# neggles/neurosis

Measured on AMD Instinct MI355X. Metric: train images/sec (node) SDXL 1024^2, higher is better.
Workload: dtype bf16

## Files before the change

include/neurosis_hip.h:

```cpp
#ifndef NEUROSIS_HIP_H
#define NEUROSIS_HIP_H

#ifdef __cplusplus
extern "C" {
#endif

const char* nk_last_error(void);
int nk_abi_version(void);

int nk_linear_fwd(const void* x, const void* w, const float* bias, const void* residual, void* y,
                  int M, int N, int K, long ldx, long ldw, long ldr, long ldy, float alpha, void* stream);
int nk_linear_dgrad(const void* dy, const void* w, const void* dx_add, void* dx, int M, int N, int K,
                    long lddy, long ldw, long ldadd, long lddx, void* stream);
long nk_linear_fwd_geglu_ok(int M, int I, int K);
int nk_linear_fwd_geglu(const void* x, const void* w, const float* bias, void* u, void* h, int M, int I, int K, long ldx, long ldw, long ldu,
                        long ldh, void* stream);
int nk_linear_dgrad_geglu(const void* dy, const void* w, const void* u, void* du, int M, int N, int I, long lddy, long ldw, long ldu,
                          long lddu, void* stream);
int nk_linear_fwd_geglu_s(const void* x, const void* w, const float* bias, void* s, void* h, int M, int I, int K, long ldx, long ldw, long lds,
                          long ldh, void* stream);
int nk_linear_dgrad_geglu_s(const void* dy, const void* w, const void* s, void* du, int M, int N, int I, long lddy, long ldw, long lds,
                            long lddu, void* stream);
int nk_linear_wgrad(const void* dy, const void* x, float* dw, int M, int N, int K, long lddy, long ldx,
                    long lddw, int accumulate, void* stream);
int nk_linear_wgrad_bias(const void* dy, const void* x, float* dw, float* dbias, int M, int N, int K, long lddy, long ldx, long lddw,
                         int accumulate, void* stream);

int nk_gemm_sk_status(void);

int nk_health_status(void);
int nk_health_clear(void);
int nk_health_export(int* dst, void* stream);
int nk_health_import(const int* src, void* stream);
int nk_debug_raise_health(void* stream);
int nk_debug_stamp(unsigned long long* dst, void* stream);
int nk_debug_launch_log(int mode);
long nk_debug_launch_names(char* buf, long cap);

int nk_colsum_batched(const void* dy, float* out, float* ws, long M, int N, long ld, int nbatch, int accumulate, void* stream);

int nk_linear_fwd_batched(const void* const* x, const void* const* w, void* const* y, int count, int M, int N, int K,
                          long ldx, long ldw, long ldy, void* stream);

int nk_linear_wgrad_batched(const void* const* dy, const void* const* x, float* const* dw, float* const* dbias, int count, int M, int N,
                            int K, long lddy, long ldx, long lddw, int accumulate, void* stream);

typedef struct NkConvDesc {
  int N, H, W, Cin;
  int Cout, KH, KW;
  int stride;
  int pad_t, pad_l;
  int Ho, Wo;
  int upsample;
} NkConvDesc;
int nk_conv2d_fwd(const NkConvDesc* d, const void* x, const void* w, const float* bias, const void* rowvec,
                  const void* residual, void* y, void* stream);
long nk_conv2d_stats_tiles(const NkConvDesc* d, int stats_groups);
int nk_conv2d_fwd_stats(const NkConvDesc* d, const void* x, const void* w, const float* bias, const void* rowvec, const void* residual,
                        void* y, float* stats_part, int stats_groups, void* stream);
int nk_conv3x3_few_channels_fwd(const void* x, const void* w, const float* bias, void* y, int N, int H, int W, int Cout, int cin_real,
                                void* stream);
int nk_conv_weight_flip(const void* w, void* wt, int Cout, int Cin, int taps, void* stream);
long nk_conv2d_dgrad_flipped_ok(const NkConvDesc* d);
int nk_conv2d_dgrad_flipped(const NkConvDesc* d, const void* dy, const void* wt, void* dx, void* stream);
int nk_conv2d_dgrad(const NkConvDesc* d, const void* dy, const void* w, void* dx, void* stream);
int nk_conv2d_wgrad(const NkConvDesc* d, const void* dy, const void* x, float* dw, int accumulate, void* stream);
int nk_conv2d_wgrad_bias(const NkConvDesc* d, const void* dy, const void* x, float* dw, float* dbias, int accumulate, void* stream);

int nk_up2_phase_weights(const void* w, void* wp, void* wd, int Cout, int Cin, void* stream);
long nk_conv2d_up2_ws_bytes(const NkConvDesc* d, int direction);
int nk_conv2d_up2_fwd(const NkConvDesc* d, const void* x, const void* wp, const float* bias, void* y, void* ws, void* stream);
int nk_conv2d_up2_dgrad(const NkConvDesc* d, const void* dy, const void* wd, void* dx, void* stream);
int nk_conv2d_up2_wgrad(const NkConvDesc* d, const void* dy, const void* x, float* dw, int accumulate, void* ws, void* stream);
int nk_conv2d_up2_wgrad_bias(const NkConvDesc* d, const void* dy, const void* x, float* dw, float* dbias, int accumulate, void* ws, void* stream);
int nk_pixel_shuffle2x(const void* phases, void* y, int N, int H, int W, int C, void* stream);
int nk_pixel_unshuffle2x(const void* y, void* phases, int N, int H, int W, int C, void* stream);
int nk_up2_fold_wgrad(const float* dwp, const float* dbias_p, float* dw, float* dbias, int Cout, int Cin, int accumulate, void* stream);

typedef struct NkAttnDesc {
  int B, H, Lq, Lk, D;
  long sq, sk, sv, so;
  long bq, bk, bv, bo;
  long sdq, sdk, sdv, sdo;
  long bdq, bdk, bdv, bdo;
  float scale;
  int causal;
} NkAttnDesc;
int nk_attention_fwd(const NkAttnDesc* d, const void* q, const void* k, const void* v, void* o, float* lse,
                     void* stream);
long nk_attention_bwd_ws_floats(const NkAttnDesc* d);
int nk_attention_bwd(const NkAttnDesc* d, const void* q, const void* k, const void* v, const void* o,
                     const float* lse, const void* d_o, void* dq, void* dk, void* dv, float* delta_ws, void* stream);
int nk_attention_bwd_causal(const NkAttnDesc* d, const void* q, const void* k, const void* v, const void* o,
                            const float* lse, const void* d_o, void* dq, void* dk, void* dv, void* stream);
int nk_attention_relbias_fwd(const NkAttnDesc* d, const void* q, const void* k, const void* v, void* o, const float* rel, void* stream);
int nk_attention_relbias_fwd_lse(const NkAttnDesc* d, const void* q, const void* k, const void* v, void* o, float* lse, const float* rel, void* stream);
long nk_attention_relbias_bwd_ws_floats(const NkAttnDesc* d);
int nk_attention_relbias_bwd(const NkAttnDesc* d, const void* q, const void* k, const void* v, const void* o, const float* lse, const void* d_o, void* dq,
                             void* dk, void* dv, const float* rel, float* d_rel, float* ws, int accumulate, void* stream);
int nk_relbias_bucket_sum(const float* d_rel, const int* buckets, float* d_weight, int H, int L, int num_buckets, int accumulate, void* stream);
int nk_softmax_rows(void* s, long M, int L, void* stream);

long nk_groupnorm_ws_floats(int N, int HW, int C, int G);
int nk_groupnorm_fwd(const void* x, const float* gamma, const float* beta, void* y, float* mean, float* rstd,
                     float* ws, int N, int HW, int C, int G, float eps, int silu, void* stream);
int nk_groupnorm_sums(const void* x, float* sums, float* ws, int N, int HW, int C, int G, void* stream);
long nk_groupnorm_sums_ws_floats(int N, int nparts, int G);
int nk_groupnorm_sums_from_parts(const float* part, float* sums, float* ws, int N, int nparts, int G, void* stream);
int nk_groupnorm_apply(const void* x, const float* sums, const float* gamma, const float* beta, void* y, float* mean, float* rstd,
                       int N, int HW, int C, int G, float eps, int silu, void* stream);
int nk_groupnorm_bwd(const void* dy, const void* x, const float* gamma, const float* beta, const float* mean,
                     const float* rstd, const void* dx_add, void* dx, float* dgamma, float* dbeta, float* ws,
                     int N, int HW, int C, int G, int silu, int accumulate, void* stream);
int nk_groupnorm_mod_fwd(const void* x, const float* gamma, const float* beta, const void* mod, void* y, float* mean, float* rstd,
                         float* ws, int N, int HW, int C, int G, float eps, int silu, void* stream);
int nk_groupnorm_mod_apply(const void* x, const float* sums, const float* gamma, const float* beta, const void* mod, void* y, float* mean,
                           float* rstd, int N, int HW, int C, int G, float eps, int silu, void* stream);
int nk_groupnorm_mod_bwd(const void* dy, const void* x, const float* gamma, const float* beta, const void* mod, const float* mean,
                         const float* rstd, const void* dx_add, void* dx, float* dgamma, float* dbeta, void* dmod, float* ws,
                         int N, int HW, int C, int G, int silu, int accumulate, void* stream);

int nk_layernorm_fwd(const void* x, const float* gamma, const float* beta, void* y, float* mean, float* rstd,
                     int M, int C, float eps, void* stream);
long nk_layernorm_ws_floats(int M, int C);
int nk_rmsnorm_fwd(const void* x, const float* gamma, void* y, int M, int C, float eps, void* stream);
int nk_rmsnorm_fwd_rstd(const void* x, const float* gamma, void* y, float* rstd, int M, int C, float eps, void* stream);
long nk_rmsnorm_bwd_ws_floats(int M, int C);
int nk_rmsnorm_bwd(const void* dy, const void* x, const float* gamma, const float* rstd, const void* dx_add, void* dx, float* dgamma, float* ws, int M, int C,
                   int accumulate, void* stream);
int nk_layernorm_bwd(const void* dy, const void* x, const float* gamma, const float* mean, const float* rstd,
                     const void* dx_add, void* dx, float* dgamma, float* dbeta, float* ws, int M, int C, int accumulate, void* stream);
#define NK_COLPART_MAX 32
typedef struct NkColpartBatch {
  const float* part[NK_COLPART_MAX];
  float* dgamma[NK_COLPART_MAX];
  float* dbeta[NK_COLPART_MAX];
  int nrows[NK_COLPART_MAX];
  int C[NK_COLPART_MAX];
  int accumulate[NK_COLPART_MAX];
  int n;
} NkColpartBatch;
long nk_layernorm_part_rows(int M);
int nk_layernorm_bwd_rows(const void* dy, const void* x, const float* gamma, const float* mean, const float* rstd,
                          const void* dx_add, void* dx, float* part, int M, int C, void* stream);
int nk_colpart_reduce_batch(const NkColpartBatch* b, void* stream);
int nk_layernorm_bwd_dx(const void* dy, const void* x, const float* gamma, const float* mean, const float* rstd,
                        const void* dx_add, void* dx, int M, int C, void* stream);
int nk_layernorm_bwd_params(const void* dy, const void* x, const float* mean, const float* rstd, float* dgamma,
                            float* dbeta, float* ws, int M, int C, int accumulate, void* stream);

int nk_geglu_fwd(const void* u, void* y, long M, int I, void* stream);
int nk_geglu_bwd(const void* dy, const void* u, void* du, long M, int I, void* stream);
int nk_geglu_fwd_s(const void* u, void* y, void* s, long M, int I, void* stream);
int nk_geglu_bwd_s(const void* dy, const void* s, void* du, long M, int I, void* stream);

int nk_silu_fwd(const void* x, void* y, long n, void* stream);
int nk_silu_bwd(const void* dy, const void* x, void* dx, long n, void* stream);

int nk_dropout(const void* x, const void* residual, void* y, long rows, int cols, long ld_x, long ld_res, long ld_y, const void* token,
               int site, int thr, float scale, void* stream);
int nk_dropout_draw(void* state, void* token, void* stream);

int nk_add(const void* a, const void* b, void* out, long n, void* stream);

int nk_cat_channels(const void* a, const void* b, void* out, long rows, int Ca, int Cb, void* stream);
int nk_split_channels(const void* src, void* a, void* b, long rows, int Ca, int Cb, void* stream);

int nk_upsample2x_bwd(const void* dup, void* dx, int N, int H, int W, int C, void* stream);
int nk_upsample2x_fwd(const void* x, void* up, int N, int H, int W, int C, void* stream);
int nk_avgpool2x_fwd(const void* x, void* y, int N, int H, int W, int C, void* stream);
int nk_avgpool2x_bwd(const void* dy, void* dx, int N, int H, int W, int C, void* stream);

int nk_nchw_to_nhwc(const void* src, int src_is_f32, void* dst, int N, int C, int HW, int Cpad, float scale,
                    void* stream);
int nk_nhwc_to_nchw(const void* src, void* dst, int dst_is_f32, int N, int C, int HW, int Cpad, void* stream);
int nk_cast_f32_to_bf16(const float* src, void* dst, long n, void* stream);
int nk_cast_bf16_to_f32(const void* src, float* dst, long n, void* stream);

long nk_colsum_ws_floats(long M, int N);
int nk_colsum(const void* dy, float* out, float* ws, long M, int N, long ld, int accumulate, void* stream);

int nk_softmax_rows_bwd(const void* p, void* dp, long M, int L, float scale, void* stream);

int nk_leaky_relu_fwd(const void* x, void* y, long n, float slope, void* stream);
int nk_leaky_relu_bwd(const void* dy, const void* y, void* dx, long n, float slope, void* stream);
long nk_batchnorm_ws_floats(long M, int C);
int nk_batchnorm_fwd(const void* x, const float* gamma, const float* beta, void* y, float* mean, float* rstd, float* running_mean,
                     float* running_var, float* ws, long M, int C, float eps, float momentum, float slope, void* stream);
int nk_batchnorm_bwd(const void* dy, const void* x, const void* y, const float* gamma, const float* mean, const float* rstd, void* dx,
                     float* dgamma, float* dbeta, float* ws, long M, int C, float slope, int accumulate, void* stream);
int nk_batchnorm_eval(const void* x, const float* gamma, const float* beta, const float* running_mean, const float* running_var, void* y,
                      float* ws, long M, int C, float eps, float slope, void* stream);

int nk_maxpool2x2_fwd(const void* x, void* y, int N, int H, int W, int C, void* stream);
int nk_maxpool2x2_bwd(const void* dy, const void* x, void* dx, int N, int H, int W, int C, void* stream);
int nk_maxpool_fwd(const void* x, void* y, int N, int H, int W, int C, int k, int s, void* stream);
// ... 124 lines not shown
```

neurosis_amd/csrc/conv_halo.h:

```cpp
#pragma once
#include <type_traits>

#ifdef NK_HALO_STAMPS
__device__ unsigned long long nk_halo_stamp_buf[8 * 8192];
__device__ unsigned long long nk_halo_kstep_buf[3 * 16 * 20 * 5];
#define CH_KSTAMP(t, ph) do { const int w_ = tid >> 6; if ((tid & 63) == 0 && (w_ == 0 || w_ == 4 || w_ == 6) && blockIdx.x >= 2048 && blockIdx.x < 2048 + 16 && (t) < 20) \
    nk_halo_kstep_buf[((((w_ == 0 ? 0 : (w_ == 4 ? 1 : 2)) * 16 + (blockIdx.x - 2048)) * 20 + (t)) * 5) + (ph)] = __builtin_amdgcn_s_memtime(); } while (0)
extern "C" int nk_debug_halo_ksteps(unsigned long long* host_out) {
  return hipMemcpyFromSymbol(host_out, HIP_SYMBOL(nk_halo_kstep_buf), sizeof(nk_halo_kstep_buf)) == hipSuccess ? 0 : 1;
}
#define CH_STAMP(slot) do { if (tid == 0 && blockIdx.x < 8192) nk_halo_stamp_buf[blockIdx.x * 8 + (slot)] = __builtin_amdgcn_s_memtime(); } while (0)
#define CH_STAMP_RT(slot) do { if (tid == 0 && blockIdx.x < 8192) nk_halo_stamp_buf[blockIdx.x * 8 + (slot)] = __builtin_amdgcn_s_memrealtime(); } while (0)
extern "C" int nk_debug_halo_stamps(unsigned long long* host_out, int nwg) {
  return hipMemcpyFromSymbol(host_out, HIP_SYMBOL(nk_halo_stamp_buf), (size_t)nwg * 8 * sizeof(unsigned long long)) == hipSuccess ? 0 : 1;
}
#else
#define CH_STAMP(slot)
#define CH_STAMP_RT(slot)
#define CH_KSTAMP(t, ph)
#endif
template <int BN_> struct HaloRing {
  static constexpr bool DEEP = BN_ == 128;
  static constexpr int BST = DEEP ? CH_BSTAGE_DEEP : CH_BSTAGE;
  static constexpr int NS = DEEP ? CH_NS_DEEP : CH_NS;
// ... 209 lines not shown
  unsigned so = 0, sn = R::AHEAD * R::BST;
  int t = 0;
  int sl = s0;
  for (int s = 0; s < nslab; ++s) {
    const unsigned hcur = lds0 + (unsigned)(s & 1) * HBUF;
    char* const hnext = smem + ((s + 1) & 1) * HBUF;
    const bool more = s + 1 < nslab;
    const int sln = sl + 1 == nslab ? 0 : sl + 1;
    const long adv_end = sl + 1 == nslab ? adv_wrap : adv_slab;
    auto step = [&](auto tapc) {
      constexpr int tap = decltype(tapc)::value;
      constexpr int dy = tap / 3, dx = tap % 3;
      __builtin_amdgcn_sched_barrier(0);
      int hpv = hpl;
      asm volatile("" : "+v"(hpv));
      g2_read<OP_KC, BN_, NJ>(bfr, fb, so);
#pragma unroll
      for (int r = 0; r < RPW; ++r) {
        const int hp = hpv + (r + dy) * CH_HW + dx;
        const unsigned ar = (unsigned)(hp * 128 + ((cl4 ^ (hp & 7)) << 4));
        const unsigned a0 = hcur + ar, a1 = hcur + (ar ^ 64u);
        G2_RD128(af[2 * r], a0, 0);
        G2_RD128(af[2 * r + 1], a0, 2048);
        G2_RD128(af[MI + 2 * r], a1, 0);
        G2_RD128(af[MI + 2 * r + 1], a1, 2048);
      }
      if constexpr (PROD) {
      } else if (hwave) {
        if (more) {
          constexpr int cnt = ch_count(HPW, HLAST, tap), st = ch_start(HPW, HLAST, tap);
#pragma unroll
          for (int i = 0; i < cnt; ++i) fire_halo(st + i, sln, hnext);
        }
        if (tap == 8) asm volatile("s_waitcnt vmcnt(0)" ::: "memory");
      } else {
        asm volatile("s_waitcnt vmcnt(0)" ::: "memory");
      }
      CH_KSTAMP(t, 4);
      CH_BAR();
      CH_KSTAMP(t, 0);
      asm volatile("s_waitcnt lgkmcnt(0)" ::: "memory");
      __builtin_amdgcn_sched_barrier(0);
      __builtin_amdgcn_s_setprio(1);
      if constexpr (!PROD) {
        if (!hwave) {
          constexpr int tap2 = (tap + 2) % 9;
          wb.fire_next(t + 2 < nk, tap2 == 8 ? adv_end : adv_tap, ring + sn, wave);
        }
      }
      CH_KSTAMP(t, 1);
#pragma unroll
      for (int ks = 0; ks < 2; ++ks)
#pragma unroll
        for (int i = 0; i < MI; ++i)
#pragma unroll
          for (int j = 0; j < NJ; ++j)
            acc[i][j] = __builtin_amdgcn_mfma_f32_16x16x32_bf16(bfr[ks * NJ + j], af[ks * MI + i], acc[i][j], 0, 0, 0);
      __builtin_amdgcn_s_setprio(0);
      CH_KSTAMP(t, 2);
      CH_BAR();
      CH_KSTAMP(t, 3);
      so += R::BST; if (so == R::NS * R::BST) so = 0;
      sn += R::BST; if (sn == R::NS * R::BST) sn = 0;
      ++t;
    };
    step(std::integral_constant<int, 0>{}); step(std::integral_constant<int, 1>{}); step(std::integral_constant<int, 2>{});
    step(std::integral_constant<int, 3>{}); step(std::integral_constant<int, 4>{}); step(std::integral_constant<int, 5>{});
    step(std::integral_constant<int, 6>{}); step(std::integral_constant<int, 7>{}); step(std::integral_constant<int, 8>{});
    sl = sln;
  }
  if (grp == 0) { CH_BAR(); }
  asm volatile("s_waitcnt vmcnt(0)" ::: "memory");
  CH_STAMP(2); CH_STAMP_RT(5);

  int mrow[MI];
  bool mok[MI];
#pragma unroll
  for (int i = 0; i < MI; ++i) {
    const int y = y0 + wq * RPW + (i >> 1), x = x0 + (i & 1) * 16 + (lane & 15);
    mok[i] = y < H && x < W;
    mrow[i] = (img * H + y) * W + x;
  }
  bf16_t* const C = (bf16_t*)p.C;
  uint4_t res8[MI][NJ / 2 ? NJ / 2 : 1];
  uint2_t res4[MI];
  if (p.residual) {
#pragma unroll
    for (int i = 0; i < MI; ++i) {
#pragma unroll
      for (int h = 0; h < NJ / 2; ++h) {
        const int n = nb + h * 32 + (g4 & 1) * 16 + (g4 >> 1) * 8;
        res8[i][h] = (mok[i] && n < Cout) ? *(const uint4_t*)(p.residual + (long)mrow[i] * p.ldr + n) : (uint4_t){0u, 0u, 0u, 0u};
      }
      if constexpr (NJ & 1) {
        const int n = nb + (NJ - 1) * 16 + g4 * 4;
        res4[i] = (mok[i] && n < Cout) ? *(const uint2_t*)(p.residual + (long)mrow[i] * p.ldr + n) : (uint2_t){0u, 0u};
      }
    }
  }
  float cadd[NJ / 2][8], cadd4[4];
#pragma unroll
  for (int h = 0; h < NJ / 2; ++h) {
    const int n = nb + h * 32 + (g4 & 1) * 16 + (g4 >> 1) * 8;
#pragma unroll
    for (int e = 0; e < 8; ++e) cadd[h][e] = 0.f;
    if (n < Cout) {
      if (p.bias) {
        const float4_t b0 = *(const float4_t*)(p.bias + n), b1 = *(const float4_t*)(p.bias + n + 4);
        cadd[h][0] = b0[0]; cadd[h][1] = b0[1]; cadd[h][2] = b0[2]; cadd[h][3] = b0[3];
        cadd[h][4] = b1[0]; cadd[h][5] = b1[1]; cadd[h][6] = b1[2]; cadd[h][7] = b1[3];
      }
      if (p.rowvec) {
        float t[8];
        unpack8(*(const uint4_t*)(p.rowvec + (long)img * p.ld_rowvec + n), t);
#pragma unroll
        for (int e = 0; e < 8; ++e) cadd[h][e] += t[e];
      }
    }
  }
#pragma unroll
  for (int e = 0; e < 4; ++e) cadd4[e] = 0.f;
  if constexpr (NJ & 1) {
    const int n = nb + (NJ - 1) * 16 + g4 * 4;
    if (n < Cout) {
      if (p.bias) { const float4_t b = *(const float4_t*)(p.bias + n); cadd4[0] = b[0]; cadd4[1] = b[1]; cadd4[2] = b[2]; cadd4[3] = b[3]; }
      if (p.rowvec) {
        float t[4];
        unpack4(*(const uint2_t*)(p.rowvec + (long)img * p.ld_rowvec + n), t);
        cadd4[0] += t[0]; cadd4[1] += t[1]; cadd4[2] += t[2]; cadd4[3] += t[3];
      }
    }
  }

  float st8[NJ / 2 ? NJ / 2 : 1][8][2], st4[4][2];
  if constexpr (STATS) {
#pragma unroll
    for (int h = 0; h < NJ / 2; ++h)
#pragma unroll
      for (int e = 0; e < 8; ++e) { st8[h][e][0] = 0.f; st8[h][e][1] = 0.f; }
#pragma unroll
    for (int e = 0; e < 4; ++e) { st4[e][0] = 0.f; st4[e][1] = 0.f; }
  }
#pragma unroll
  for (int i = 0; i < MI; ++i) {
#pragma unroll
    for (int h = 0; h < NJ / 2; ++h) {
      float v[8];
#pragma unroll
      for (int r = 0; r < 4; ++r) {
        const float a_own = acc[i][2 * h][r], b_own = acc[i][2 * h + 1][r];
        auto sw = __builtin_amdgcn_permlane16_swap(__float_as_uint(a_own), __float_as_uint(b_own), false, false);
        v[r] = __uint_as_float(sw[0]);
        v[4 + r] = __uint_as_float(sw[1]);
      }
      const int n = nb + h * 32 + (g4 & 1) * 16 + (g4 >> 1) * 8;
#pragma unroll
      for (int e = 0; e < 8; ++e) v[e] += cadd[h][e];
      if (p.residual) {
        float tr[8];
        unpack8(res8[i][h], tr);
#pragma unroll
        for (int e = 0; e < 8; ++e) v[e] += tr[e];
      }
      const uint4_t packed = pack8(v);
      const bool ok = mok[i] && n < Cout;
      if (ok) *(uint4_t*)(C + (long)mrow[i] * p.ldc + n) = packed;
      if constexpr (STATS) {
        float q[8];
        unpack8(packed, q);
#pragma unroll
        for (int e = 0; e < 8; ++e) { const float x = ok ? q[e] : 0.f; st8[h][e][0] += x; st8[h][e][1] += x * x; }
      }
    }
    if constexpr (NJ & 1) {
      const int n = nb + (NJ - 1) * 16 + g4 * 4;
      float v[4] = {acc[i][NJ - 1][0] + cadd4[0], acc[i][NJ - 1][1] + cadd4[1], acc[i][NJ - 1][2] + cadd4[2], acc[i][NJ - 1][3] + cadd4[3]};
      if (p.residual) {
        float tr[4];
        unpack4(res4[i], tr);
        v[0] += tr[0]; v[1] += tr[1]; v[2] += tr[2]; v[3] += tr[3];
      }
      uint2_t o;
      o.x = pack2bf(v[0], v[1]);
      o.y = pack2bf(v[2], v[3]);
      const bool ok = mok[i] && n < Cout;
      if (ok) *(uint2_t*)(C + (long)mrow[i] * p.ldc + n) = o;
      if constexpr (STATS) {
        float q[4];
        unpack4(o, q);
#pragma unroll
        for (int e = 0; e < 4; ++e) { const float x = ok ? q[e] : 0.f; st4[e][0] += x; st4[e][1] += x * x; }
      }
    }
  }
  if constexpr (STATS) {
    __syncthreads();
    float* const cs = (float*)ring;
    auto lane16_sum = [](float x) {
      x += __builtin_bit_cast(float, __builtin_amdgcn_update_dpp(0, __builtin_bit_cast(int, x), 0xB1, 0xF, 0xF, true));
      x += __builtin_bit_cast(float, __builtin_amdgcn_update_dpp(0, __builtin_bit_cast(int, x), 0x4E, 0xF, 0xF, true));
      x += __builtin_bit_cast(float, __builtin_amdgcn_update_dpp(0, __builtin_bit_cast(int, x), 0x141, 0xF, 0xF, true));
      x += __builtin_bit_cast(float, __builtin_amdgcn_update_dpp(0, __builtin_bit_cast(int, x), 0x140, 0xF, 0xF, true));
      return x;
    };
#pragma unroll
    for (int h = 0; h < NJ / 2; ++h)
#pragma unroll
      for (int e = 0; e < 8; ++e)
#pragma unroll
        for (int k = 0; k < 2; ++k) {
          const float tot = lane16_sum(st8[h][e][k]);
          const int col = h * 32 + (g4 & 1) * 16 + (g4 >> 1) * 8 + e;
          if ((lane & 15) == 0) cs[(wave * HN + col) * 2 + k] = tot;
        }
    if constexpr (NJ & 1) {
#pragma unroll
      for (int e = 0; e < 4; ++e)
#pragma unroll
        for (int k = 0; k < 2; ++k) {
          const float tot = lane16_sum(st4[e][k]);
          const int col = (NJ - 1) * 16 + g4 * 4 + e;
          if ((lane & 15) == 0) cs[(wave * HN + col) * 2 + k] = tot;
        }
    }
    __syncthreads();
    const int cpg = Cout / p.stats_groups;
    const int ngt = BN_ / cpg;
    if (tid < 2 * ngt) {
      const int gi = tid >> 1, k = tid & 1;
      float a = 0.f;
      for (int cc = 0; cc < cpg; ++cc) {
        const int col = gi * cpg + cc;
        const int gh = col / HN, cl = col - gh * HN;
#pragma unroll
        for (int w4 = 0; w4 < 4; ++w4) a += cs[((gh * 4 + w4) * HN + cl) * 2 + k];
      }
      p.stats_part[((long)img * per_img + trem) * 2 * p.stats_groups + 2 * (n0 / cpg + gi) + k] = a;
    }
  }
#ifdef NK_HALO_STAMPS
  asm volatile("s_waitcnt vmcnt(0)" ::: "memory");
  CH_STAMP(3);
#endif
#undef CH_BAR
}
```

neurosis_amd/csrc/gemm.hip:

```cpp
#include "nk_common.h"
#include "nk_gemm.h"
#include "gemm_plan.h"

#define NTHREADS 256
#define KC_IMAGE_BYTES (128 * 128)
#define MC_ROW_BYTES (128 * 2 + 16)
#define MC_IMAGE_BYTES (BK * MC_ROW_BYTES)
#define OPND_BYTES MC_IMAGE_BYTES
#define STAGE_BYTES (2 * OPND_BYTES)
#define SMEM_BYTES (2 * STAGE_BYTES)

static_assert(SMEM_BYTES >= BM * CS_LD * 4, "epilogue staging must fit");

__device__ __forceinline__ bool is_kc(int mode) { return mode == OP_KC || mode == OP_KCG; }

__device__ __forceinline__ long gather_offset(const NkGather& g, int n, int bh, int bw, int kh, int kw,
                                              int c, bool& valid) {
  int hn = bh + kh * g.ks;
  int wn = bw + kw * g.ks;
  bool ok = (hn >= 0) & (wn >= 0);
  ok &= (((hn | wn) & g.need_even) == 0);
  const int sh = g.div >> 1;
  int h = hn >> sh, w = wn >> sh;
  ok &= (h < g.H) & (w < g.W);
// ... 1306 lines not shown
    for (int q = 0; q < 2; ++q) {
      ba[q] = p.bias ? *(const float4_t*)(p.bias + abase + q * 16 + cl) : (float4_t){0.f, 0.f, 0.f, 0.f};
      bg[q] = p.bias ? *(const float4_t*)(p.bias + I + abase + q * 16 + cl) : (float4_t){0.f, 0.f, 0.f, 0.f};
    }
    NkGemmParams ph = p;
    ph.N = I; ph.ldc = p.ld_h; ph.bias = nullptr;
    NkGemmParams ps = p;
    ps.bias = nullptr;
#pragma unroll
    for (int ib = 0; ib < 2; ++ib) {
      float4_t pa[4][2], pg[4][2], phh[4][2];
#pragma unroll
      for (int i = 0; i < 4; ++i)
#pragma unroll
        for (int q = 0; q < 2; ++q) {
          pa[i][q] = acc[ib * 4 + i][2 * q];
          pg[i][q] = acc[ib * 4 + i][2 * q + 1];
#pragma unroll
          for (int r = 0; r < 4; ++r) {
            const float av = bf2f(f2bf(pa[i][q][r] + ba[q][r])), gv = bf2f(f2bf(pg[i][q][r] + bg[q][r]));
            float cdf, pdf;
            normal_cdf_pdf(gv, cdf, pdf);
            const float ge = gv * cdf;
            phh[i][q][r] = av * ge;
            if (p.geglu_save) {
              pa[i][q][r] = ge;
              pg[i][q][r] = av * (cdf + gv * pdf);
            }
          }
        }
      const int mb = m0 + wm * 128 + ib * 64;
      if (p.geglu_save) {
        reg_epilogue_64x32<0>(ps, p.C, pa, mb, abase, lane);
        reg_epilogue_64x32<0>(ps, p.C, pg, mb, I + abase, lane);
      } else {
        reg_epilogue_64x32<0>(p, p.C, pa, mb, abase, lane);
        reg_epilogue_64x32<0>(p, p.C, pg, mb, I + abase, lane);
      }
      reg_epilogue_64x32<0>(ph, p.geglu_h, phh, mb, abase, lane);
    }
    return;
  }
#pragma unroll
  for (int ib = 0; ib < 2; ++ib)
#pragma unroll
    for (int half = 0; half < 2; ++half) {
      float4_t pair[4][2];
#pragma unroll
      for (int i = 0; i < 4; ++i) { pair[i][0] = acc[ib * 4 + i][2 * half]; pair[i][1] = acc[ib * 4 + i][2 * half + 1]; }
      reg_epilogue_64x32<0>(p, p.C, pair, m0 + wm * 128 + ib * 64, n0 + wn * 64 + half * 32, lane);
    }
}

__global__ void nk_zero_f32_kernel(float* __restrict__ dst, size_t n);
#include "gemm_g2.h"
#include "gemm_w160.h"
#include "conv_halo.h"
#include "conv_wgrad_halo.h"

typedef void (*NkGemmKernel)(const NkGemmParams);
static int launch_plan(NkGemmKernel kern, const NkGemmPlan& pl, const NkGemmParams& p, hipStream_t stream) {
  nk_optin_lds((const void*)kern, pl.smem);
  hipLaunchKernelGGL(kern, dim3(pl.grid[0], pl.grid[1], pl.grid[2]), dim3(pl.block), pl.smem, stream, p);
  return nk_check_launch(pl.name);
}

template <int A_, int B_, int F32_> struct Modes { static constexpr int A = A_, B = B_, F32 = F32_; };
template <class Fn>
static int with_modes(int amode, int bmode, int out_f32, Fn f) {
#define NK_CASE(A_, B_) \
  if (amode == A_ && bmode == B_) return out_f32 ? f(Modes<A_, B_, 1>()) : f(Modes<A_, B_, 0>());
  NK_CASE(OP_KC, OP_KC)
  NK_CASE(OP_KC, OP_MC)
  NK_CASE(OP_MC, OP_MC)
  NK_CASE(OP_KCG, OP_KC)
  NK_CASE(OP_KCG, OP_MCT)
  NK_CASE(OP_MC, OP_MCG)
#undef NK_CASE
  nk_set_error(__FILE__, __LINE__, "unsupported operand mode combination");
  return NK_ERR_ARG;
}

static NkGemmKernel halo_kernel(const NkGemmPlan& pl) {
  if (pl.bn == 160) {
    if (pl.halo_rows == 8) return pl.flag ? nk_conv3x3_halo_kernel<160, 4, 1> : nk_conv3x3_halo_kernel<160, 4, 0>;
    return pl.flag ? nk_conv3x3_halo_kernel<160, 2, 1> : nk_conv3x3_halo_kernel<160, 2, 0>;
  }
  if (pl.halo_rows == 8) return pl.flag ? nk_conv3x3_halo_kernel<128, 4, 1> : nk_conv3x3_halo_kernel<128, 4, 0>;
  return pl.flag ? nk_conv3x3_halo_kernel<128, 2, 1> : nk_conv3x3_halo_kernel<128, 2, 0>;
}

#include <mutex>
#include <unordered_map>
struct SkWorkspace {
  unsigned* flags = nullptr;
  float* ws = nullptr;
};
static std::mutex sk_mutex;
static std::unordered_map<void*, SkWorkspace> sk_spaces;

static int sk_prepare(NkGemmParams& p, hipStream_t stream) {
  std::lock_guard<std::mutex> lock(sk_mutex);
  SkWorkspace& w = sk_spaces[(void*)stream];
  if (!w.ws) {
    hipStreamCaptureStatus capturing = hipStreamCaptureStatusNone;
    if (hipStreamIsCapturing(stream, &capturing) == hipSuccess && capturing != hipStreamCaptureStatusNone) {
      nk_set_error(__FILE__, __LINE__, "stream-K workspace requested while the stream is capturing: run the launch once on this stream before capturing it");
      return NK_ERR_LAUNCH;
    }
    char* raw = nullptr;
    const size_t ws_bytes = (size_t)SK_MAX_GRID * SK_TILE_FLOATS * sizeof(float);
    if (hipMalloc((void**)&raw, ws_bytes + (SK_MAX_GRID + 64) * sizeof(unsigned)) != hipSuccess) {
      nk_set_error(__FILE__, __LINE__, "hipMalloc of the stream-K workspace failed");
      return NK_ERR_LAUNCH;
    }
    w.ws = (float*)raw;
    w.flags = (unsigned*)(raw + ws_bytes);
    if (hipMemsetAsync(w.flags, 0, (SK_MAX_GRID + 64) * sizeof(unsigned), stream) != hipSuccess) return NK_ERR_LAUNCH;
  }
  p.sk_health = nk_health_word();
  if (!p.sk_health) { nk_set_error(__FILE__, __LINE__, "health word allocation failed"); return NK_ERR_LAUNCH; }
  p.sk_flags = w.flags;
  p.sk_ws = w.ws;
  return NK_OK;
}

int nk_gemm_sk_reset(void) {
  std::lock_guard<std::mutex> lock(sk_mutex);
  for (auto& kv : sk_spaces)
    if (kv.second.flags && hipMemset(kv.second.flags, 0, (SK_MAX_GRID + 64) * sizeof(unsigned)) != hipSuccess) return NK_ERR_LAUNCH;
  return NK_OK;
}

extern "C" int nk_gemm_sk_status(void) {
  std::lock_guard<std::mutex> lock(sk_mutex);
  if (hipDeviceSynchronize() != hipSuccess) return -1;
  int bad = 0;
  for (auto& kv : sk_spaces) {
    unsigned v = 0;
    if (kv.second.flags && hipMemcpy(&v, kv.second.flags + SK_MAX_GRID + 1, sizeof(v), hipMemcpyDeviceToHost) == hipSuccess && v) bad = 1;
  }
  return bad;
}

__global__ __launch_bounds__(256) void nk_zero_f32_kernel(float* __restrict__ dst, size_t n) {
  const size_t n4 = n / 4, stride = (size_t)gridDim.x * 256;
  float4_t* d4 = (float4_t*)dst;
  for (size_t i = (size_t)blockIdx.x * 256 + threadIdx.x; i < n4; i += stride) d4[i] = (float4_t){0.f, 0.f, 0.f, 0.f};
  if (blockIdx.x == 0 && threadIdx.x < (n & 3)) dst[n4 * 4 + threadIdx.x] = 0.f;
}

static int zero_split_outputs(const NkGemmParams& p, hipStream_t stream) {
  for (int z = 0; z < (p.nbatch ? p.nbatch : 1); ++z) {
    const size_t n = (size_t)p.M * p.N;
    float* dst = (float*)(p.nbatch ? p.Cb[z] : p.C);
    const unsigned blocks = (unsigned)((n / 4 + 255) / 256 > 2048 ? 2048 : (n / 4 + 255) / 256);
    hipLaunchKernelGGL(nk_zero_f32_kernel, dim3(blocks ? blocks : 1), dim3(256), 0, stream, dst, n);
    float* db = p.nbatch ? p.dbias_b[z] : p.dbias;
    if (db) hipLaunchKernelGGL(nk_zero_f32_kernel, dim3(1), dim3(256), 0, stream, db, (size_t)p.M);
  }
  return hipGetLastError() != hipSuccess ? NK_ERR_LAUNCH : NK_OK;
}

int nk_gemm_dispatch(NkGemmParams& p, int amode, int bmode, int out_f32, int allow_splitk,
                     hipStream_t stream) {
  NK_CHECK_ARG(p.M > 0 && p.N > 0 && p.K > 0);
  if (!p.nbatch) NK_CHECK_ARG(((uintptr_t)p.A & 15) == 0 && ((uintptr_t)p.B & 15) == 0 && ((uintptr_t)p.C & 15) == 0);
  for (int z = 0; z < p.nbatch; ++z) NK_CHECK_ARG(((uintptr_t)p.Ab[z] & 15) == 0 && ((uintptr_t)p.Bb[z] & 15) == 0 && ((uintptr_t)p.Cb[z] & 15) == 0);
  if (amode == OP_KC) NK_CHECK_ARG((p.K & 7) == 0 && (p.lda & 7) == 0);
  if (bmode == OP_KC) NK_CHECK_ARG((p.K & 7) == 0 && (p.ldb & 7) == 0);
  if (amode == OP_KCG) NK_CHECK_ARG((p.ga.C & 7) == 0);
  if (amode == OP_MC) NK_CHECK_ARG((p.M & 7) == 0 && (p.lda & 7) == 0);
  if (bmode == OP_MC) NK_CHECK_ARG((p.N & 7) == 0 && (p.ldb & 7) == 0);
  if (bmode == OP_MCT) NK_CHECK_ARG((p.N & 7) == 0 && (p.tw.co_stride & 7) == 0 && (p.tw.tap_stride & 7) == 0);
  if (bmode == OP_MCG) NK_CHECK_ARG((p.gb.C & 7) == 0);
  if (p.residual) NK_CHECK_ARG(((uintptr_t)p.residual & 15) == 0 && ((p.ldr & 7) == 0 || (p.N & 7) != 0));
  if (!out_f32) NK_CHECK_ARG((p.ldc & 7) == 0 || (p.N & 7) != 0);
  if (p.fRowsPerBatch.d == 0) p.fRowsPerBatch = make_fastdiv(1);

  if (p.dbias || (p.nbatch && p.dbias_b[0])) NK_CHECK_ARG(amode == OP_MC && out_f32);
  if (p.geglu_h) {
    NK_CHECK_ARG(amode == OP_KC && bmode == OP_KC && !out_f32 && !p.nbatch && (p.N & 255) == 0 && (p.ld_h & 7) == 0 && !p.rowvec && !p.residual && p.alpha == 1.0f);
    NK_CHECK_ARG(((uintptr_t)p.geglu_h & 15) == 0 && (!p.bias || ((uintptr_t)p.bias & 15) == 0));
  } else if (p.geglu_u) {
    NK_CHECK_ARG(amode == OP_KC && bmode == OP_MC && !out_f32 && !p.nbatch && (p.N & 7) == 0 && (p.ld_u & 7) == 0 && !p.bias && !p.rowvec && !p.residual);
  }

  const TileEnv env = tile_env();
  const NkGemmPlan pl = nk_gemm_plan(p, amode, bmode, out_f32, allow_splitk, env);
  if (pl.err) {
    nk_set_error(__FILE__, __LINE__, pl.err);
    return NK_ERR_ARG;
  }
  if (pl.zero_c) NK_CHECK_ARG(p.ldc == p.N);
  const int logging = nk_launch_log_mode();
  char line[192];
  if (logging) nk_plan_line(pl, line, sizeof(line));
  if (logging == 3) {
    nk_launch_log_add(pl.name, line);
    return NK_OK;
  }

  p.ksplit_len = pl.ksplit_len; p.accumulate = pl.accumulate; p.k_rotate = pl.k_rotate; p.group_m = pl.group_m; p.sk_chunked = pl.sk_chunked;
  if (pl.zero_c)
    if (int rc = zero_split_outputs(p, stream)) return rc;
  if (pl.family == NK_FAM_SK) {
    p.sk_debug = env.sk_debug;
    if (int rc = sk_prepare(p, stream)) return rc;
  }

  int rc;
  switch (pl.family) {
    case NK_FAM_HALO: rc = launch_plan(halo_kernel(pl), pl, p, stream); break;
    case NK_FAM_WGRAD_HALO: rc = launch_plan(pl.flag ? nk_conv3x3_wgrad_halo_kernel<1> : nk_conv3x3_wgrad_halo_kernel<0>, pl, p, stream); break;
    case NK_FAM_W160: rc = launch_plan(pl.bn == 160 ? nk_gemm_w160_kernel<160> : nk_gemm_w160_kernel<128>, pl, p, stream); break;
    case NK_FAM_RING64: rc = launch_plan(nk_gemm_ring64_kernel, pl, p, stream); break;
    case NK_FAM_XL: rc = launch_plan(nk_gemm_xl_kernel<OP_KCG, 64, 64>, pl, p, stream); break;
    case NK_FAM_XL2G: rc = launch_plan(pl.flag ? nk_gemm_xl2g_kernel<OP_KC, 1> : nk_gemm_xl2g_kernel<OP_KC, 0>, pl, p, stream); break;
    case NK_FAM_G2P:
      rc = with_modes(amode, bmode, out_f32, [&](auto m) {
        using M = decltype(m);
        if constexpr (M::B == OP_MCG) return (int)NK_ERR_ARG;
        else return launch_plan(pl.bn == 160 ? nk_gemm_g2p_kernel<M::A, M::B, M::F32, 160> : nk_gemm_g2p_kernel<M::A, M::B, M::F32, 128>, pl, p, stream);
      });
      break;
    case NK_FAM_SK:
      rc = with_modes(amode, bmode, out_f32, [&](auto m) { using M = decltype(m); return launch_plan(nk_gemm_sk_kernel<M::A, M::B, M::F32>, pl, p, stream); });
      break;
    case NK_FAM_RING:
      rc = with_modes(amode, bmode, out_f32, [&](auto m) { using M = decltype(m); return launch_plan(nk_gemm_ring_kernel<M::A, M::B, M::F32>, pl, p, stream); });
      break;
    case NK_FAM_DMA:
      rc = with_modes(amode, bmode, out_f32, [&](auto m) { using M = decltype(m); return launch_plan(nk_gemm_dma_kernel<M::A, M::B, M::F32, 8>, pl, p, stream); });
      break;
    default:
      nk_set_error(__FILE__, __LINE__, "the plan names no kernel");
      return NK_ERR_ARG;
  }
  if (logging) nk_launch_log_add(nullptr, line);
  return rc;
}

int nk_halo_tiles_per_image(const NkGemmParams& p, int* bn) {
  const NkGemmPlan pl = nk_gemm_plan(p, OP_KCG, OP_KC, 0, 0, tile_env());
  if (pl.err || pl.family != NK_FAM_HALO) return 0;
  if (bn) *bn = pl.bn;
  return pl.tiles_per_image;
}

int nk_geglu_fwd_fusable(const NkGemmParams& p) {
  if (p.N & 255) return 0;
  const NkGemmPlan pl = nk_gemm_plan(p, OP_KC, OP_KC, 0, 0, tile_env());
  return !pl.err && pl.family == NK_FAM_XL2G && pl.flag ? 1 : 0;
}
```

neurosis_amd/csrc/gemm_plan.h:

```cpp
#pragma once
#include "nk_gemm.h"
#include <stdio.h>
#include <stdlib.h>

enum { OP_KC = 0, OP_KCG = 1, OP_MC = 2, OP_MCT = 3, OP_MCG = 4 };

#define BM 128
#define BN 128
#define BK 64
#define GROUP_M 8
#define CS_LD 132
#define V2_OPND_BYTES 16384
#define V2_STAGE_BYTES (2 * V2_OPND_BYTES)
#define V2_SMEM_BYTES (BM * CS_LD * 4)
#define RING_NS 4
#define RING_SMEM_BYTES (RING_NS * V2_STAGE_BYTES)
#define SK_NT 512
#define SK_SMEM_BYTES (2 * V2_STAGE_BYTES)
#define SK_MAX_GRID 512
#define R64_NS 8
#define R64_OPND 8192
#define R64_STAGE (2 * R64_OPND)
#define R64_SMEM (R64_NS * R64_STAGE)
#define XL_BM 256
// ... 212 lines not shown
  }
  if (!((amode == OP_KC && bmode == OP_KC) || (amode == OP_KC && bmode == OP_MC) || (amode == OP_MC && bmode == OP_MC) ||
        (conv && (bmode == OP_KC || bmode == OP_MCT))))
    return false;
  if (p.K < 2 * BK) return false;
  if (amode == OP_MC && bmode == OP_MC && !p.nbatch) return false;
  const int bn = g2_bn(p.N);
  if (!bn) return false;
  if (mode == 2) return true;
  const long tiles = (long)((p.M + G2_BM - 1) / G2_BM) * ((p.N + bn - 1) / bn) * (p.nbatch ? p.nbatch : 1);
  const long rounds = (tiles + 255) / 256;
  const double fill = (double)tiles / (double)(rounds * 256);
  const long nk = (p.K + BK - 1) / BK;
  if (fill < 0.85) return false;
  return rounds <= 2 || (rounds <= 4 && nk >= 40);
}

static bool use_sk(const TileEnv& env, const NkGemmParams& p, int out_f32) {
  const int mode = env.sk;
  if (mode == 0) return false;
  if (mode == 1) return true;
  if (mode == 2) return out_f32 != 0;
  if (mode == 4 && out_f32) return false;
  const long tiles = (long)((p.M + BM - 1) / BM) * ((p.N + BN - 1) / BN) * (p.nbatch ? p.nbatch : 1);
  const long nk = (p.K + BK - 1) / BK;
  const long rounds = (tiles + 511) / 512;
  const double fill = (double)tiles / (double)(rounds * 512);
  if (tiles >= 1024 && fill >= 0.8) return false;
  if (tiles >= 512 && fill >= 0.95) return false;
  return nk >= 24;
}

static int pick_splitk(int M, int N, int K, int max_split) {
  int tiles = ((M + BM - 1) / BM) * ((N + BN - 1) / BN);
  int nk = (K + BK - 1) / BK;
  const int lo = 96, hi = 192;
  if (tiles >= lo && tiles * 2 <= 512 && nk >= 256 && max_split >= 2) return 2;
  if (tiles >= lo) return 1;
  int s = 1;
  while (s < max_split && tiles * s < hi && nk / (s * 2) >= 8) s *= 2;
  return s;
}

static void plan_kernel(NkGemmPlan& pl, int family, const char* name, long gx, int gy, int gz, int block, int smem) {
  pl.family = family; pl.name = name;
  pl.grid[0] = (unsigned)gx; pl.grid[1] = (unsigned)gy; pl.grid[2] = (unsigned)gz;
  pl.block = block; pl.smem = smem;
}
static void plan_split(NkGemmPlan& pl, const NkGemmParams& p, int splits) {
  pl.splitk = splits;
  pl.ksplit_len = cdiv(cdiv(p.K, BK), splits) * BK;
  if (splits > 1 && pl.accumulate == 0) {
    pl.zero_c = true; pl.zero_dbias = has_dbias(p);
    pl.accumulate = 1;
  } else if (pl.accumulate == 2) {
    pl.accumulate = splits > 1 ? 1 : 0;
  }
}
static void plan_xl(NkGemmPlan& pl, const TileEnv& env, const NkGemmParams& p, int amode) {
  const long tiles = (long)cdiv(p.M, XL_BM) * cdiv(p.N, XL_BN);
  if (amode == OP_KC) {
    pl.flag = p.geglu_h != nullptr;
    plan_kernel(pl, NK_FAM_XL2G, pl.flag ? "nk_gemm_xl2g_kernel<geglu=1>" : "nk_gemm_xl2g_kernel<geglu=0>", tiles, 1, 1, 512, XL_SMEM_BYTES);
    pl.k_rotate = k_rotate_on(env, p.K);
  } else {
    plan_kernel(pl, NK_FAM_XL, "nk_gemm_xl_kernel", tiles, 1, 1, 1024, XL_SMEM_BYTES);
  }
}
static void plan_ring_or_dma(NkGemmPlan& pl, const TileEnv& env, const NkGemmParams& p) {
  const int ntm = cdiv(p.M, BM), ntn = cdiv(p.N, BN);
  {
    int per_xcd = (ntm * ntn + 7) / 8, g = 1;
    while ((g + 1) * (g + 1) <= per_xcd) ++g;
    pl.group_m = g > GROUP_M ? GROUP_M : g;
  }
  pl.k_rotate = k_rotate_on(env, pl.splitk > 1 ? pl.ksplit_len : p.K);
  if (!p.nbatch && (long)ntm * ntn * pl.splitk <= 256) plan_kernel(pl, NK_FAM_RING, "nk_gemm_ring_kernel", ntm * ntn, pl.splitk, 1, 512, RING_SMEM_BYTES);
  else plan_kernel(pl, NK_FAM_DMA, "nk_gemm_dma_kernel", ntm * ntn, pl.splitk, nbatch1(p), 512, V2_SMEM_BYTES);
}
static const char* halo_name(int bn, int rows, int stats) {
  static const char* const names[2][2][2] = {
      {{"nk_conv3x3_halo_kernel<128,4,stats=0>", "nk_conv3x3_halo_kernel<128,4,stats=1>"}, {"nk_conv3x3_halo_kernel<128,8,stats=0>", "nk_conv3x3_halo_kernel<128,8,stats=1>"}},
      {{"nk_conv3x3_halo_kernel<160,4,stats=0>", "nk_conv3x3_halo_kernel<160,4,stats=1>"}, {"nk_conv3x3_halo_kernel<160,8,stats=0>", "nk_conv3x3_halo_kernel<160,8,stats=1>"}}};
  return names[bn == 160][rows == 8][stats != 0];
}

static NkGemmPlan nk_gemm_plan(const NkGemmParams& p, int amode, int bmode, int out_f32, int allow_splitk, const TileEnv& env) {
  NkGemmPlan pl = {};
  pl.splitk = 1;
  pl.ksplit_len = p.ksplit_len; pl.accumulate = p.accumulate; pl.k_rotate = p.k_rotate; pl.group_m = p.group_m; pl.sk_chunked = p.sk_chunked;

  if (p.geglu_h) {
    if (amode != OP_KC || !use_xl(env, p, amode, bmode, out_f32, 1)) {
      pl.err = "fused GEGLU forward on a shape the 256 x 256 kernel does not take (ask nk_linear_fwd_geglu_ok first)";
      return pl;
    }
    plan_split(pl, p, 1);
    plan_xl(pl, env, p, OP_KC);
    return pl;
  }
  if (p.geglu_u) {
    plan_split(pl, p, 1);
    plan_ring_or_dma(pl, env, p);
    return pl;
  }
  if (use_halo(env, p, amode, bmode, out_f32)) {
    const NkGather& g = p.ga;
    pl.bn = halo_bn(p.N); pl.halo_rows = halo_tile_rows(p); pl.flag = p.stats_part != nullptr;
    pl.tiles_per_image = cdiv(g.W, CH_TW) * cdiv(g.H, pl.halo_rows);
    plan_kernel(pl, NK_FAM_HALO, halo_name(pl.bn, pl.halo_rows, pl.flag), (long)p.halo_nb * pl.tiles_per_image * (p.N / pl.bn), 1, 1,
                halo_threads(pl.bn), halo_smem(pl.bn, pl.halo_rows));
    pl.k_rotate = k_rotate_on(env, g.C);
    return pl;
  }
  if (use_wgrad_halo(env, p, amode, bmode, out_f32)) {
    int per = 0;
    const int S = wgrad_halo_splits(p, per);
    const long nblk = (long)((p.M + WH_BCO - 1) / WH_BCO) * (p.gb.C / WH_BCI);
    pl.flag = p.dbias != nullptr;
    plan_kernel(pl, NK_FAM_WGRAD_HALO, pl.flag ? "nk_conv3x3_wgrad_halo_kernel<bias=1>" : "nk_conv3x3_wgrad_halo_kernel<bias=0>", nblk * S, 1, 1, 512, WH_SMEM);
    pl.splitk = S;
    pl.ksplit_len = per;
    pl.zero_c = S > 1 && p.accumulate == 0; pl.zero_dbias = pl.zero_c && p.dbias;
    pl.accumulate = p.accumulate == 1 ? 1 : 0;
    return pl;
  }
  if (p.stats_part) {
    pl.err = "statistics epilogue on a convolution the halo-tile kernel does not take (ask nk_conv2d_stats_tiles first)";
    return pl;
  }

  {
    const W160Plan wp = w160_plan(env, p, amode, bmode, out_f32, allow_splitk);
    if (wp.bn) {
      pl.bn = wp.bn;
      plan_split(pl, p, wp.splitk);
      pl.k_rotate = k_rotate_on(env, wp.splitk > 1 ? pl.ksplit_len : p.K);
      plan_kernel(pl, NK_FAM_W160, wp.bn == 160 ? "nk_gemm_w160_kernel<160>" : "nk_gemm_w160_kernel<128>", (long)cdiv(p.M, W160_BM) * cdiv(p.N, wp.bn),
                  wp.splitk, nbatch1(p), 512, w160_smem(wp.bn));
      return pl;
    }
  }
  if (use_ring64(env, p, amode, bmode, out_f32)) {
    plan_kernel(pl, NK_FAM_RING64, "nk_gemm_ring64_kernel", (long)((p.M + 63) >> 6) * ((p.N + 63) >> 6), 1, 1, 512, R64_SMEM);
    return pl;
  }
  if ((!p.nbatch || p.nbatch <= NK_MAX_BATCH) && use_g2(env, p, amode, bmode, out_f32, 1) && (env.g2 == 2 || !use_xl(env, p, amode, bmode, out_f32, 1))) {
    pl.bn = g2_bn(p.N);
    if (pl.accumulate == 2) pl.accumulate = 0;
    pl.k_rotate = k_rotate_on(env, p.K);
    plan_kernel(pl, NK_FAM_G2P, pl.bn == 160 ? "nk_gemm_g2p_kernel<160>" : "nk_gemm_g2p_kernel<128>", (long)cdiv(p.M, G2_BM) * cdiv(p.N, pl.bn), 1, nbatch1(p), 768,
                G2_SMEM_BYTES);
    return pl;
  }

  if (!has_dbias(p) && use_sk(env, p, out_f32)) {
    const long T = (long)cdiv(p.M, BM) * cdiv(p.N, BN) * nbatch1(p), W = T * cdiv(p.K, BK);
    if (W < (1l << 22)) {
      if (pl.accumulate == 2) pl.accumulate = 0;
      const int max_grid = SK_MAX_GRID & ~7, min_iters = 4;
      long grid = (W / min_iters) & ~7l;
      if (grid > max_grid) grid = max_grid;
      if (grid < 8) grid = 8;
      pl.sk_chunked = T >= 64;
      plan_kernel(pl, NK_FAM_SK, "nk_gemm_sk_kernel", grid, 1, 1, SK_NT, SK_SMEM_BYTES);
      return pl;
    }
  }
  if (p.nbatch > NK_MAX_BATCH) { pl.err = "p.nbatch <= NK_MAX_BATCH"; return pl; }
  plan_split(pl, p, out_f32 && allow_splitk ? pick_splitk(p.M * nbatch1(p), p.N, p.K, 32) : 1);
  if (use_xl(env, p, amode, bmode, out_f32, pl.splitk)) {
    plan_xl(pl, env, p, amode);
    return pl;
  }
  const bool known = (amode == OP_KC && (bmode == OP_KC || bmode == OP_MC)) || (amode == OP_MC && (bmode == OP_MC || bmode == OP_MCG)) ||
                     (amode == OP_KCG && (bmode == OP_KC || bmode == OP_MCT));
  if (!known) { pl.err = "unsupported operand mode combination"; return pl; }
  plan_ring_or_dma(pl, env, p);
  return pl;
}
```

neurosis_amd/csrc/nk_gemm.h:

```cpp
#pragma once
#include "nk_common.h"

struct NkGather {
  int H, W, C;
  int Ho, Wo;
  int KW;
  int rs, ks;
  int off_h, off_w;
  int div;
  int need_even;
  FastDiv fWo, fHoWo, fC, fKW;
};

struct NkTapW {
  long co_stride, tap_stride;
  FastDiv fCout;
};

struct NkGemmParams {
  const bf16_t* A;
  const bf16_t* B;
  long lda, ldb;
  int M, N, K;
  NkGather ga, gb;
  NkTapW tw;
  void* C;
  long ldc;
  float alpha;
  int sk_debug;
  const float* bias;
  const bf16_t* residual;
  long ldr;
  const bf16_t* rowvec;
  long ld_rowvec;
  FastDiv fRowsPerBatch;
  int ksplit_len;
  int group_m;
  int accumulate;
  int sk_chunked;
  int k_rotate;
  int nbatch;
  const bf16_t* Ab[8];
  const bf16_t* Bb[8];
  void* Cb[8];
  unsigned* sk_flags;
  float* sk_ws;
  unsigned* sk_health;
  float* dbias;
  float* dbias_b[8];
  const bf16_t* geglu_u;
  long ld_u;
  bf16_t* geglu_h;
  long ld_h;
  int geglu_save;
  int halo_nb;
  float* stats_part;
  int stats_groups;
};
#define NK_MAX_BATCH 8

enum { NK_OP_KC = 0, NK_OP_KCG = 1, NK_OP_MC = 2, NK_OP_MCT = 3, NK_OP_MCG = 4 };

int nk_gemm_dispatch(NkGemmParams& p, int amode, int bmode, int out_f32, int allow_splitk, hipStream_t stream);
int nk_halo_tiles_per_image(const NkGemmParams& p, int* bn);
int nk_geglu_fwd_fusable(const NkGemmParams& p);
```

neurosis_amd/csrc/norm.hip:

```cpp
#include "../../include/neurosis_hip.h"
#include "nk_common.h"
#include "nk_reduce.h"
#include "norm_plan.h"
#include <type_traits>

__global__ __launch_bounds__(GN_THREADS) void gn_stats_kernel(const bf16_t* __restrict__ x, float* __restrict__ stats,
                                                              int HW, int C, int G, int rows_per) {
  __shared__ float ps[GN_THREADS * 8], pss[GN_THREADS * 8];
  const int n = blockIdx.y;
  const int cpr = (C >> 3) / gridDim.z;
  const int ch0 = blockIdx.z * cpr;
  const int rows_par = GN_THREADS / cpr;
  const int tid = threadIdx.x;
  const int cpg = C / G;
  const int row_lo = blockIdx.x * rows_per;
  const int row_hi = min(HW, row_lo + rows_per);
  float s[8], ss[8];
#pragma unroll
  for (int e = 0; e < 8; ++e) { s[e] = 0.f; ss[e] = 0.f; }
  const int chunk = tid % cpr, rsub = tid / cpr;
  if (rsub < rows_par) {
    const bf16_t* base = x + ((long)n * HW) * C + (ch0 + chunk) * 8;
    int r = row_lo + rsub;
    for (; r + 3 * rows_par < row_hi; r += 4 * rows_par) {
// ... 301 lines not shown
  for (; i + GN_THREADS < total; i += 2 * GN_THREADS) {
    uint4_t vx[2], vd[2], va[2];
#pragma unroll
    for (int u = 0; u < 2; ++u) {
      const size_t o = off0 + (size_t)(i + u * GN_THREADS) * 8;
      vx[u] = *(const uint4_t*)(x + o);
      vd[u] = *(const uint4_t*)(dy + o);
      va[u] = dx_add ? *(const uint4_t*)(dx_add + o) : zero4;
    }
#pragma unroll
    for (int u = 0; u < 2; ++u) one(i + u * GN_THREADS, vx[u], vd[u], va[u]);
  }
  for (; i < total; i += GN_THREADS) {
    const size_t o = off0 + (size_t)i * 8;
    one(i, *(const uint4_t*)(x + o), *(const uint4_t*)(dy + o), dx_add ? *(const uint4_t*)(dx_add + o) : zero4);
  }
}

static int gn_forward(int pass, bool modulated, const void* x, float* sums, const float* gamma, const float* beta, const void* mod, void* y, float* mean,
                      float* rstd, float* ws, int N, int HW, int C, int G, float eps, int silu, void* stream_) {
  hipStream_t stream = (hipStream_t)stream_;
  const NkGnPlan p = nk_gn_plan(N, HW, C, G, pass, modulated);
  NORM_PLAN_OR_RETURN(p);
  NK_CHECK_ARG(x && (pass == GN_APPLY || ws) && (pass == GN_FWD || sums) && (pass == GN_SUMS || (gamma && beta && y && mean && rstd)) && (!modulated || mod));
  if (pass == GN_FWD) sums = ws + p.gsum.off;
  for (int i = 0; i < p.n; ++i) {
    const NkNormLaunch& L = p.launch[i];
    if (L.kernel == NK_GN_STATS) NORM_LAUNCH(L, gn_stats_kernel, (const bf16_t*)x, ws + p.part.off, HW, C, G, p.rows_per);
    else if (L.kernel == NK_GN_REDUCE) NORM_LAUNCH(L, gn_reduce_partials_kernel, ws + p.part.off, sums, p.nparts, 2 * G);
    else if (modulated) NORM_LAUNCH(L, gn_apply_kernel<true>, (const bf16_t*)x, sums, gamma, beta, (const bf16_t*)mod, (bf16_t*)y, mean, rstd, HW, C, G, eps, silu, p.rows_per);
    else NORM_LAUNCH(L, gn_apply_kernel<false>, (const bf16_t*)x, sums, gamma, beta, (const bf16_t*)nullptr, (bf16_t*)y, mean, rstd, HW, C, G, eps, silu, p.rows_per);
    if (int e = nk_check_launch(L.name)) return e;
  }
  return NK_OK;
}

static int gn_backward(bool modulated, const void* dy_, const void* x_, const float* gamma, const float* beta, const void* mod_, const float* mean, const float* rstd,
                       const void* dx_add, void* dx, float* dgamma, float* dbeta, void* dmod, float* ws, int N, int HW, int C, int G, int silu, int accumulate,
                       void* stream_) {
  hipStream_t stream = (hipStream_t)stream_;
  const NkGnPlan p = nk_gn_plan(N, HW, C, G, GN_BWD, modulated);
  NORM_PLAN_OR_RETURN(p);
  NK_CHECK_ARG(dy_ && x_ && gamma && beta && mean && rstd && dx && dgamma && dbeta && ws && (!modulated || (mod_ && dmod)));
  const bf16_t *dy = (const bf16_t*)dy_, *x = (const bf16_t*)x_, *mod = (const bf16_t*)mod_;
  float *part = ws + p.part.off, *gsum = ws + p.gsum.off, *chan = ws + p.chan.off;
  for (int i = 0; i < p.n; ++i) {
    const NkNormLaunch& L = p.launch[i];
    switch (L.kernel) {
      case NK_GN_BWD_STATS:
        if (modulated) NORM_LAUNCH(L, gn_bwd_stats_kernel<true>, dy, x, gamma, beta, mod, mean, rstd, part, chan, HW, C, G, silu, p.rows_per);
        else NORM_LAUNCH(L, gn_bwd_stats_kernel<false>, dy, x, gamma, beta, mod, mean, rstd, part, chan, HW, C, G, silu, p.rows_per);
        break;
      case NK_GN_REDUCE: NORM_LAUNCH(L, gn_reduce_partials_kernel, part, gsum, p.nparts, 2 * G); break;
      case NK_GN_COLPART: NORM_LAUNCH(L, colpart_reduce_kernel, chan, dgamma, dbeta, p.chan_rows, C, accumulate); break;
      case NK_GN_COLPART_MOD: NORM_LAUNCH(L, colpart_reduce_mod_kernel, chan, mod, dgamma, dbeta, p.chan_rows, p.nsplit, C, accumulate); break;
      case NK_GN_DMOD: NORM_LAUNCH(L, gn_dmod_kernel, chan, gamma, beta, (bf16_t*)dmod, p.nsplit, C); break;
      case NK_GN_BWD_APPLY:
        if (modulated) NORM_LAUNCH(L, gn_bwd_apply_kernel<true>, dy, x, gamma, beta, mod, mean, rstd, gsum, (const bf16_t*)dx_add, (bf16_t*)dx, HW, C, G, silu, p.rows_per);
        else NORM_LAUNCH(L, gn_bwd_apply_kernel<false>, dy, x, gamma, beta, mod, mean, rstd, gsum, (const bf16_t*)dx_add, (bf16_t*)dx, HW, C, G, silu, p.rows_per);
        break;
    }
    if (int e = nk_check_launch(L.name)) return e;
  }
  return NK_OK;
}

extern "C" long nk_groupnorm_ws_floats(int N, int HW, int C, int G) { return nk_gn_plan(N, HW, C, G, GN_BWD, false).ws_floats; }

extern "C" int nk_groupnorm_fwd(const void* x, const float* gamma, const float* beta, void* y, float* mean, float* rstd, float* ws, int N, int HW, int C, int G, float eps,
                                int silu, void* stream) {
  return gn_forward(GN_FWD, false, x, nullptr, gamma, beta, nullptr, y, mean, rstd, ws, N, HW, C, G, eps, silu, stream);
}
extern "C" int nk_groupnorm_sums(const void* x, float* sums, float* ws, int N, int HW, int C, int G, void* stream) {
  return gn_forward(GN_SUMS, false, x, sums, nullptr, nullptr, nullptr, nullptr, nullptr, nullptr, ws, N, HW, C, G, 0.f, 0, stream);
}
extern "C" int nk_groupnorm_apply(const void* x, const float* sums, const float* gamma, const float* beta, void* y, float* mean, float* rstd, int N, int HW, int C, int G,
                                  float eps, int silu, void* stream) {
  return gn_forward(GN_APPLY, false, x, (float*)sums, gamma, beta, nullptr, y, mean, rstd, nullptr, N, HW, C, G, eps, silu, stream);
}
extern "C" int nk_groupnorm_bwd(const void* dy, const void* x, const float* gamma, const float* beta, const float* mean, const float* rstd, const void* dx_add, void* dx,
                                float* dgamma, float* dbeta, float* ws, int N, int HW, int C, int G, int silu, int accumulate, void* stream) {
  return gn_backward(false, dy, x, gamma, beta, nullptr, mean, rstd, dx_add, dx, dgamma, dbeta, nullptr, ws, N, HW, C, G, silu, accumulate, stream);
}
extern "C" int nk_groupnorm_mod_fwd(const void* x, const float* gamma, const float* beta, const void* mod, void* y, float* mean, float* rstd, float* ws, int N, int HW,
                                    int C, int G, float eps, int silu, void* stream) {
  return gn_forward(GN_FWD, true, x, nullptr, gamma, beta, mod, y, mean, rstd, ws, N, HW, C, G, eps, silu, stream);
}
extern "C" int nk_groupnorm_mod_apply(const void* x, const float* sums, const float* gamma, const float* beta, const void* mod, void* y, float* mean, float* rstd, int N,
                                      int HW, int C, int G, float eps, int silu, void* stream) {
  return gn_forward(GN_APPLY, true, x, (float*)sums, gamma, beta, mod, y, mean, rstd, nullptr, N, HW, C, G, eps, silu, stream);
}
extern "C" int nk_groupnorm_mod_bwd(const void* dy, const void* x, const float* gamma, const float* beta, const void* mod, const float* mean, const float* rstd,
                                    const void* dx_add, void* dx, float* dgamma, float* dbeta, void* dmod, float* ws, int N, int HW, int C, int G, int silu,
                                    int accumulate, void* stream) {
  return gn_backward(true, dy, x, gamma, beta, mod, mean, rstd, dx_add, dx, dgamma, dbeta, dmod, ws, N, HW, C, G, silu, accumulate, stream);
}

__global__ __launch_bounds__(256) void gn_reduce_partials_l1_kernel(const float* __restrict__ part, float* __restrict__ out, int nparts, int G2, int nchunks) {
  __shared__ float sm[4][64];
  const int n = blockIdx.y, chunk = blockIdx.x;
  const int tx = threadIdx.x & 63, ty = threadIdx.x >> 6;
  float a = 0.f;
  if (tx < G2)
    for (int p = chunk + ty * nchunks; p < nparts; p += 4 * nchunks) a += part[((long)n * nparts + p) * G2 + tx];
  sm[ty][tx] = a;
  __syncthreads();
  if (ty == 0 && tx < G2) out[((long)n * nchunks + chunk) * G2 + tx] = (a + sm[1][tx]) + (sm[2][tx] + sm[3][tx]);
}

extern "C" long nk_groupnorm_sums_ws_floats(int N, int nparts, int G) { return nk_gn_sums_plan(N, nparts, G).ws_floats; }
extern "C" int nk_groupnorm_sums_from_parts(const float* part, float* sums, float* ws, int N, int nparts, int G, void* stream_) {
  hipStream_t stream = (hipStream_t)stream_;
  const NkGnSumsPlan p = nk_gn_sums_plan(N, nparts, G);
  NORM_PLAN_OR_RETURN(p);
  NK_CHECK_ARG(part && sums && (p.levels == 1 || ws));
  for (int i = 0; i < p.n; ++i) {
    const NkNormLaunch& L = p.launch[i];
    if (L.kernel == NK_GN_REDUCE_L1) {
      NORM_LAUNCH(L, gn_reduce_partials_l1_kernel, part, ws + p.l1.off, nparts, 2 * G, p.nchunks);
      part = ws + p.l1.off;
      nparts = p.nchunks;
    } else {
      NORM_LAUNCH(L, gn_reduce_partials_kernel, part, sums, nparts, 2 * G);
    }
    if (int e = nk_check_launch(L.name)) return e;
  }
  return NK_OK;
}

template <int NCH>
__global__ __launch_bounds__(256) void ln_fwd_kernel(const bf16_t* __restrict__ x, const float* __restrict__ gamma,
                                                     const float* __restrict__ beta, bf16_t* __restrict__ y,
                                                     float* __restrict__ mean, float* __restrict__ rstd, int M, int C,
                                                     float eps) {
  const int lane = threadIdx.x & 63;
  const int wave = (blockIdx.x * blockDim.x + threadIdx.x) >> 6;
  const int nwaves = (gridDim.x * blockDim.x) >> 6;
  const int cpr = C >> 3;
  const float invC = 1.0f / (float)C;
  for (int row = wave; row < M; row += nwaves) {
    float f[NCH][8];
    float s = 0.f;
#pragma unroll
    for (int j = 0; j < NCH; ++j) {
      int ch = lane + 64 * j;
      if (ch < cpr) {
        unpack8(*(const uint4_t*)(x + (long)row * C + ch * 8), f[j]);
#pragma unroll
        for (int e = 0; e < 8; ++e) s += f[j][e];
      }
    }
    const float mu = wave_sum(s) * invC;
    float v = 0.f;
#pragma unroll
    for (int j = 0; j < NCH; ++j) {
      int ch = lane + 64 * j;
      if (ch < cpr) {
#pragma unroll
        for (int e = 0; e < 8; ++e) { float d = f[j][e] - mu; v += d * d; }
      }
    }
    const float rs = rsqrtf(wave_sum(v) * invC + eps);
    if (lane == 0) { mean[row] = mu; rstd[row] = rs; }
#pragma unroll
    for (int j = 0; j < NCH; ++j) {
      int ch = lane + 64 * j;
// ... 484 lines not shown
```

neurosis_amd/csrc/norm_plan.h:

```cpp
#pragma once
#include "../../include/neurosis_hip.h"
#include <stdio.h>

#define GN_THREADS 256
#define GN_MAXC 4096
#define GN_MAXG 64
#define GN_SUMS_MAXG 32
#define GN_SUMS_ONE_LEVEL 128
#define GN_SUMS_CHUNKS 64
#define LN_MAXCH 4
#define RMS_MAXCH 8
#define ROWNORM_MAX_BLOCKS 4096
#define LNP_ROWS 64
#define LNR_WAVES 4
#define LNR_MAX_BLOCKS 512
#define LNR_MAX_SMEM (2 * 2 * 2048 * 4)
#define RMSB_MAX_ROWS 512
#define CS_ROWS 64
#define CS_MAX_SPLIT 1024
#define NORM_WS_PAD 64

enum NormKernel {
  NK_GN_STATS, NK_GN_REDUCE, NK_GN_REDUCE_L1, NK_GN_APPLY, NK_GN_BWD_STATS, NK_GN_COLPART, NK_GN_COLPART_MOD, NK_GN_DMOD, NK_GN_BWD_APPLY,
  NK_LN_FWD, NK_LN_BWD_DX, NK_LN_BWD_PARAM, NK_LN_BWD_ROWS, NK_LN_COLPART, NK_RMS_FWD, NK_COLPART_BATCH, NK_CS_PARTIAL, NK_CS_REDUCE,
  NK_RMS_BWD_ROWS, NK_RMS_COLPART
};
struct NkNormRegion { const char* name; long off, len; };
struct NkNormLaunch {
  int kernel;
  const char* name;
  unsigned grid[3];
  int block, smem;
  NkNormRegion reg[2];
};
struct NkNormPlan {
  int n;
  NkNormLaunch launch[5];
  long ws_floats;
  const char* err;
};

static inline NkNormLaunch& norm_launch(NkNormPlan& pl, int kernel, const char* name, unsigned x, unsigned y, unsigned z, int block, int smem,
                                 NkNormRegion r0 = {nullptr, 0, 0}, NkNormRegion r1 = {nullptr, 0, 0}) {
  NkNormLaunch& L = pl.launch[pl.n++];
  L.kernel = kernel; L.name = name; L.block = block; L.smem = smem;
  L.grid[0] = x; L.grid[1] = y; L.grid[2] = z;
  L.reg[0] = r0; L.reg[1] = r1;
  return L;
}

static inline void nk_norm_plan_line(const NkNormPlan& pl, int i, char* buf, size_t cap) {
  const NkNormLaunch& L = pl.launch[i];
  int at = snprintf(buf, cap, "%s grid=%u,%u,%u %d %d", L.name, L.grid[0], L.grid[1], L.grid[2], L.block, L.smem);
  for (int r = 0; r < 2 && at > 0 && (size_t)at < cap; ++r)
    if (L.reg[r].len) at += snprintf(buf + at, cap - at, " %s=%ld+%ld", L.reg[r].name, L.reg[r].off, L.reg[r].len);
  if (at > 0 && (size_t)at < cap) snprintf(buf + at, cap - at, " ws=%ld", pl.ws_floats);
}
static inline void nk_norm_plan_log(const NkNormPlan& pl, void (*add)(const char*, const char*)) {
  char line[192];
  for (int i = 0; i < pl.n; ++i) {
    nk_norm_plan_line(pl, i, line, sizeof(line));
    add(pl.launch[i].name, line);
  }
}

enum GnPass { GN_FWD, GN_SUMS, GN_APPLY, GN_BWD };
struct NkGnPlan : NkNormPlan {
  int rows_per, nsplit, nz;
  int nparts, chan_rows;
  NkNormRegion part, gsum, chan;
};
static inline NkGnPlan nk_gn_plan(int N, int HW, int C, int G, int pass, bool mod) {
  NkGnPlan p = {};
  if (!(N > 0 && HW > 0 && C > 0 && G > 0 && G <= GN_MAXG)) { p.err = "N > 0 && HW > 0 && C > 0 && G > 0 && G <= 64"; return p; }
  if (!((C & 7) == 0 && C % G == 0 && C <= GN_MAXC)) { p.err = "(C & 7) == 0 && C % G == 0 && C <= GN_MAXC"; return p; }
  const int cpr = C >> 3;
  p.nz = (cpr + GN_THREADS - 1) / GN_THREADS;
  while (cpr % p.nz) ++p.nz;
  const int want = (1024 + N - 1) / N;
  p.rows_per = (HW + want - 1) / want;
  if (p.rows_per < 32) p.rows_per = 32;
  p.nsplit = (HW + p.rows_per - 1) / p.rows_per;
  p.nparts = p.nsplit * p.nz;
  p.chan_rows = N * p.nsplit;
  p.part = {"part", 0, (long)N * p.nparts * 2 * G};
  p.gsum = {"gsum", p.part.len, (long)N * 2 * G};
  p.chan = {"chan", p.gsum.off + p.gsum.len, (long)p.chan_rows * 2 * C};
  p.ws_floats = p.chan.off + p.chan.len + NORM_WS_PAD;
  const int smem2 = 2 * C * (int)sizeof(float);
  const unsigned ns = (unsigned)p.nsplit, n = (unsigned)N, cb = (unsigned)((C + 63) / 64);
  if (pass == GN_FWD || pass == GN_SUMS) {
    norm_launch(p, NK_GN_STATS, "gn_stats_kernel", ns, n, (unsigned)p.nz, GN_THREADS, 0, p.part);
    norm_launch(p, NK_GN_REDUCE, "gn_reduce_partials_kernel", n, 1, 1, 1024, 0, p.part, pass == GN_FWD ? p.gsum : NkNormRegion{nullptr, 0, 0});
  }
  if (pass == GN_FWD || pass == GN_APPLY)
    norm_launch(p, NK_GN_APPLY, mod ? "gn_apply_kernel<mod>" : "gn_apply_kernel", ns, n, 1, GN_THREADS, smem2,
                pass == GN_FWD ? p.gsum : NkNormRegion{nullptr, 0, 0});
  if (pass == GN_BWD) {
    norm_launch(p, NK_GN_BWD_STATS, mod ? "gn_bwd_stats_kernel<mod>" : "gn_bwd_stats_kernel", ns, n, (unsigned)p.nz, GN_THREADS, smem2, p.part, p.chan);
    norm_launch(p, NK_GN_REDUCE, "gn_reduce_partials_kernel", n, 1, 1, 1024, 0, p.part, p.gsum);
    if (mod) {
      norm_launch(p, NK_GN_COLPART_MOD, "colpart_reduce_mod_kernel", cb, 1, 1, 1024, 0, p.chan);
      norm_launch(p, NK_GN_DMOD, "gn_dmod_kernel", cb, n, 1, 1024, 0, p.chan);
    } else {
      norm_launch(p, NK_GN_COLPART, "colpart_reduce_kernel", cb, 1, 1, 1024, 0, p.chan);
    }
    norm_launch(p, NK_GN_BWD_APPLY, mod ? "gn_bwd_apply_kernel<mod>" : "gn_bwd_apply_kernel", ns, n, 1, GN_THREADS, 2 * smem2, p.gsum);
  }
  return p;
}

struct NkGnSumsPlan : NkNormPlan {
  int levels, nchunks;
  NkNormRegion l1;
};
static inline NkGnSumsPlan nk_gn_sums_plan(int N, int nparts, int G) {
  NkGnSumsPlan p = {};
  if (!(N > 0 && nparts > 0 && G > 0 && G <= GN_SUMS_MAXG)) { p.err = "N > 0 && nparts > 0 && G > 0 && G <= 32"; return p; }
  p.nchunks = GN_SUMS_CHUNKS;
  p.levels = nparts > GN_SUMS_ONE_LEVEL ? 2 : 1;
  p.l1 = {"l1", 0, p.levels == 2 ? (long)N * p.nchunks * 2 * G : 0};
  p.ws_floats = (long)N * p.nchunks * 2 * G + NORM_WS_PAD;
  if (p.levels == 2) norm_launch(p, NK_GN_REDUCE_L1, "gn_reduce_partials_l1_kernel", (unsigned)p.nchunks, (unsigned)N, 1, 256, 0, p.l1);
  norm_launch(p, NK_GN_REDUCE, "gn_reduce_partials_kernel", (unsigned)N, 1, 1, 1024, 0, p.l1);
  return p;
}

enum RowNormKind { LN_FWD, LN_BWD_DX, LN_BWD_PARAMS, LN_BWD_ROWS, LN_BWD, RMS_FWD, RMS_FWD_RSTD, RMS_BWD };
struct NkRowNormPlan : NkNormPlan {
  int nch;
  int part_rows;
  int param_split;
  int nrows;
  NkNormRegion part;
};
static inline NkRowNormPlan nk_rownorm_plan(int M, int C, int kind) {
  NkRowNormPlan p = {};
  const bool rms = kind == RMS_FWD || kind == RMS_FWD_RSTD || kind == RMS_BWD;
  const int maxch = rms ? RMS_MAXCH : LN_MAXCH;
  if (!(M > 0 && C > 0 && (C & 7) == 0)) { p.err = "M > 0 && C > 0 && (C & 7) == 0"; return p; }
  const int need = ((C >> 3) + 63) / 64;
  if (kind == LN_BWD_PARAMS) p.nch = 0;
  else if (rms) p.nch = need <= 2 ? 2 : (need <= 4 ? 4 : 8);
  else p.nch = need <= 2 ? 2 : need;
  p.param_split = (M + LNP_ROWS - 1) / LNP_ROWS;
  p.part_rows = (M + 4 * LNR_WAVES - 1) / (4 * LNR_WAVES);
  if (p.part_rows > LNR_MAX_BLOCKS) p.part_rows = LNR_MAX_BLOCKS;
  const unsigned rowgrid = (unsigned)((M + 3) / 4 < ROWNORM_MAX_BLOCKS ? (M + 3) / 4 : ROWNORM_MAX_BLOCKS), cb = (unsigned)((C + 63) / 64);
  const bool has_ws = kind == LN_BWD_PARAMS || kind == LN_BWD_ROWS || kind == LN_BWD;
  p.nrows = !has_ws ? 0 : (kind == LN_BWD_PARAMS ? p.param_split : p.part_rows);
  p.part = {"part", 0, (long)p.nrows * 2 * C};
  p.ws_floats = !has_ws ? 0 : kind == LN_BWD_ROWS ? p.part.len : (long)(p.param_split > LNR_MAX_BLOCKS ? p.param_split : LNR_MAX_BLOCKS) * 2 * C + NORM_WS_PAD;
  if (kind != LN_BWD_PARAMS && (C >> 3) > 64 * maxch) { p.err = rms ? "(C >> 3) <= 64 * RMS_MAXCH" : "(C >> 3) <= 64 * LN_MAXCH"; return p; }
  if (kind == RMS_BWD) {
    p.nrows = M < RMSB_MAX_ROWS ? M : RMSB_MAX_ROWS;
    p.part = {"part", 0, (long)p.nrows * C};
    p.ws_floats = p.part.len + NORM_WS_PAD;
    norm_launch(p, NK_RMS_BWD_ROWS, "rms_bwd_rows_kernel", (unsigned)((p.nrows + 3) / 4), 1, 1, 256, 0, p.part);
    norm_launch(p, NK_RMS_COLPART, "rms_colpart_reduce_kernel", cb, 1, 1, 1024, 0, p.part);
    return p;
  }
  if (kind == LN_FWD) norm_launch(p, NK_LN_FWD, "ln_fwd_kernel", rowgrid, 1, 1, 256, 0);
  if (kind == RMS_FWD || kind == RMS_FWD_RSTD) norm_launch(p, NK_RMS_FWD, "rms_fwd_kernel", rowgrid, 1, 1, 256, 0);
  if (kind == LN_BWD_DX) norm_launch(p, NK_LN_BWD_DX, "ln_bwd_dx_kernel", rowgrid, 1, 1, 256, 0);
  if (kind == LN_BWD_PARAMS) norm_launch(p, NK_LN_BWD_PARAM, "ln_bwd_param_kernel", (unsigned)p.param_split, (unsigned)((C + 127) / 128), 1, 256, 0, p.part);
  if (kind == LN_BWD_ROWS || kind == LN_BWD)
    norm_launch(p, NK_LN_BWD_ROWS, "ln_bwd_rows_kernel", (unsigned)p.part_rows, 1, 1, LNR_WAVES * 64, 2 * 2 * C * (int)sizeof(float), p.part);
  if (kind == LN_BWD_PARAMS || kind == LN_BWD) norm_launch(p, NK_LN_COLPART, "colpart_reduce_kernel", cb, 1, 1, 1024, 0, p.part);
  return p;
}

static inline NkNormPlan nk_colpart_batch_plan(const int* C, int n) {
  NkNormPlan p = {};
  if (!(n > 0 && n <= NK_COLPART_MAX)) { p.err = "b->n > 0 && b->n <= NK_COLPART_MAX"; return p; }
  int maxC = 0;
  for (int z = 0; z < n; ++z) {
    if (C[z] <= 0) { p.err = "b->C[z] > 0"; return p; }
    maxC = C[z] > maxC ? C[z] : maxC;
  }
  norm_launch(p, NK_COLPART_BATCH, "colpart_reduce_batch_kernel", (unsigned)((maxC + 31) / 32), (unsigned)n, 1, 1024, 0);
  return p;
}

struct NkColsumPlan : NkNormPlan {
  int rows_per_block, nsplit;
  NkNormRegion part;
};
static inline NkColsumPlan nk_colsum_plan(long M, int N, int nbatch) {
  NkColsumPlan p = {};
  if (!(M > 0 && N > 0 && (N & 7) == 0 && nbatch >= 1 && nbatch <= 65535)) { p.err = "M > 0 && N > 0 && (N & 7) == 0 && nbatch >= 1 && nbatch <= 65535"; return p; }
  long rows = CS_ROWS;
// ... 10 lines not shown
```

neurosis_amd/csrc/ops_gemm.hip:

```cpp
#include "../../include/neurosis_hip.h"
#include "nk_gemm.h"
#include <string.h>

static NkGemmParams zero_params() {
  NkGemmParams p;
  memset(&p, 0, sizeof(p));
  p.alpha = 1.0f;
  p.fRowsPerBatch = make_fastdiv(1);
  p.ga.fWo = p.ga.fHoWo = p.ga.fC = p.ga.fKW = make_fastdiv(1);
  p.gb.fWo = p.gb.fHoWo = p.gb.fC = p.gb.fKW = make_fastdiv(1);
  p.tw.fCout = make_fastdiv(1);
  return p;
}

extern "C" int nk_linear_fwd(const void* x, const void* w, const float* bias, const void* residual, void* y,
                             int M, int N, int K, long ldx, long ldw, long ldr, long ldy, float alpha,
                             void* stream) {
  NkGemmParams p = zero_params();
  p.A = (const bf16_t*)x; p.lda = ldx;
  p.B = (const bf16_t*)w; p.ldb = ldw;
  p.M = M; p.N = N; p.K = K;
  p.C = y; p.ldc = ldy;
  p.bias = bias;
  p.residual = (const bf16_t*)residual; p.ldr = ldr;
  p.alpha = alpha;
  return nk_gemm_dispatch(p, NK_OP_KC, NK_OP_KC, 0, 0, (hipStream_t)stream);
}

extern "C" int nk_linear_fwd_batched(const void* const* x, const void* const* w, void* const* y, int count, int M, int N, int K,
                                     long ldx, long ldw, long ldy, void* stream) {
  NK_CHECK_ARG(x && w && y && count >= 1 && count <= NK_MAX_BATCH);
  NkGemmParams p = zero_params();
  p.lda = ldx; p.ldb = ldw;
  p.M = M; p.N = N; p.K = K;
  p.ldc = ldy;
  p.nbatch = count;
  for (int i = 0; i < count; ++i) {
    p.Ab[i] = (const bf16_t*)x[i];
    p.Bb[i] = (const bf16_t*)w[i];
    p.Cb[i] = y[i];
  }
  p.A = p.Ab[0]; p.B = p.Bb[0]; p.C = p.Cb[0];
  return nk_gemm_dispatch(p, NK_OP_KC, NK_OP_KC, 0, 0, (hipStream_t)stream);
}

extern "C" int nk_linear_dgrad(const void* dy, const void* w, const void* dx_add, void* dx, int M, int N, int K,
                               long lddy, long ldw, long ldadd, long lddx, void* stream) {
  NkGemmParams p = zero_params();
  p.A = (const bf16_t*)dy; p.lda = lddy;
  p.B = (const bf16_t*)w; p.ldb = ldw;
  p.M = M; p.N = K; p.K = N;
  p.C = dx; p.ldc = lddx;
  p.residual = (const bf16_t*)dx_add; p.ldr = ldadd;
  return nk_gemm_dispatch(p, NK_OP_KC, NK_OP_MC, 0, 0, (hipStream_t)stream);
}

static NkGemmParams geglu_fwd_params(const void* x, const void* w, const float* bias, void* u, void* h, int M, int I, int K, long ldx, long ldw,
                                      long ldu, long ldh) {
  NkGemmParams p = zero_params();
  p.A = (const bf16_t*)x; p.lda = ldx;
  p.B = (const bf16_t*)w; p.ldb = ldw;
  p.M = M; p.N = 2 * I; p.K = K;
  p.C = u; p.ldc = ldu;
  p.bias = bias;
  p.geglu_h = (bf16_t*)h; p.ld_h = ldh;
  return p;
}
extern "C" long nk_linear_fwd_geglu_ok(int M, int I, int K) {
  if (M <= 0 || I <= 0 || K <= 0 || (I & 127) || (K & 7)) return 0;
  NkGemmParams p = geglu_fwd_params(nullptr, nullptr, nullptr, nullptr, (void*)16, M, I, K, K, K, 2l * I, I);
  return nk_geglu_fwd_fusable(p);
}
extern "C" int nk_linear_fwd_geglu(const void* x, const void* w, const float* bias, void* u, void* h, int M, int I, int K, long ldx, long ldw,
                                   long ldu, long ldh, void* stream) {
  NK_CHECK_ARG(x && w && u && h && M > 0 && I > 0 && K > 0);
  NkGemmParams p = geglu_fwd_params(x, w, bias, u, h, M, I, K, ldx, ldw, ldu, ldh);
  return nk_gemm_dispatch(p, NK_OP_KC, NK_OP_KC, 0, 0, (hipStream_t)stream);
}

extern "C" int nk_linear_fwd_geglu_s(const void* x, const void* w, const float* bias, void* s, void* h, int M, int I, int K, long ldx, long ldw,
                                     long lds, long ldh, void* stream) {
  NK_CHECK_ARG(x && w && s && h && M > 0 && I > 0 && K > 0);
  NkGemmParams p = geglu_fwd_params(x, w, bias, s, h, M, I, K, ldx, ldw, lds, ldh);
  p.geglu_save = 1;
// ... 89 lines not shown
  return g;
}

static NkGemmParams conv_fwd_params(const NkConvDesc* d, const void* x, const void* w, const float* bias, const void* rowvec,
                                    const void* residual, void* y) {
  NkGemmParams p = zero_params();
  p.A = (const bf16_t*)x;
  p.ga = fwd_gather(d);
  p.B = (const bf16_t*)w; p.ldb = (long)d->KH * d->KW * d->Cin;
  p.M = d->N * d->Ho * d->Wo; p.N = d->Cout; p.K = d->KH * d->KW * d->Cin;
  p.C = y; p.ldc = d->Cout;
  p.bias = bias;
  p.rowvec = (const bf16_t*)rowvec; p.ld_rowvec = d->Cout;
  p.fRowsPerBatch = make_fastdiv(d->Ho * d->Wo);
  p.residual = (const bf16_t*)residual; p.ldr = d->Cout;
  p.halo_nb = (d->KH == 3 && d->KW == 3) ? d->N : 0;
  return p;
}

extern "C" int nk_conv2d_fwd(const NkConvDesc* d, const void* x, const void* w, const float* bias,
                             const void* rowvec, const void* residual, void* y, void* stream) {
  if (int e = check_conv(d)) return e;
  NkGemmParams p = conv_fwd_params(d, x, w, bias, rowvec, residual, y);
  return nk_gemm_dispatch(p, NK_OP_KCG, NK_OP_KC, 0, 0, (hipStream_t)stream);
}

extern "C" long nk_conv2d_stats_tiles(const NkConvDesc* d, int stats_groups) {
  if (check_conv(d)) return 0;
  if (stats_groups < 0 || stats_groups > 32) return 0;
  NkGemmParams p = conv_fwd_params(d, nullptr, nullptr, nullptr, nullptr, nullptr, nullptr);
  int bn = 0;
  const int tiles = nk_halo_tiles_per_image(p, &bn);
  if (tiles && stats_groups) {
    if (d->Cout % stats_groups) return 0;
    if (bn % (d->Cout / stats_groups)) return 0;
  }
  return tiles;
}

extern "C" int nk_conv2d_fwd_stats(const NkConvDesc* d, const void* x, const void* w, const float* bias, const void* rowvec,
                                   const void* residual, void* y, float* stats_part, int stats_groups, void* stream) {
  if (int e = check_conv(d)) return e;
  NK_CHECK_ARG(stats_part && stats_groups > 0);
  NK_CHECK_ARG(nk_conv2d_stats_tiles(d, stats_groups) > 0);
  NkGemmParams p = conv_fwd_params(d, x, w, bias, rowvec, residual, y);
  p.stats_part = stats_part; p.stats_groups = stats_groups;
  return nk_gemm_dispatch(p, NK_OP_KCG, NK_OP_KC, 0, 0, (hipStream_t)stream);
}

extern "C" int nk_conv2d_dgrad(const NkConvDesc* d, const void* dy, const void* w, void* dx, void* stream) {
  if (int e = check_conv(d)) return e;
  const int Hin = d->upsample ? 2 * d->H : d->H, Win = d->upsample ? 2 * d->W : d->W;
  NkGemmParams p = zero_params();
  NkGather g;
  memset(&g, 0, sizeof(g));
  g.H = d->Ho; g.W = d->Wo; g.C = d->Cout;
  g.Ho = Hin; g.Wo = Win; g.KW = d->KW;
  g.rs = 1; g.ks = -1;
  g.off_h = d->pad_t; g.off_w = d->pad_l;
  g.div = d->stride; g.need_even = d->stride - 1;
  g.fWo = make_fastdiv(Win); g.fHoWo = make_fastdiv(Hin * Win);
  g.fC = make_fastdiv(d->Cout); g.fKW = make_fastdiv(d->KW);
  p.A = (const bf16_t*)dy; p.ga = g;
  p.B = (const bf16_t*)w;
  p.tw.co_stride = (long)d->KH * d->KW * d->Cin;
  p.tw.tap_stride = d->Cin;
  p.tw.fCout = make_fastdiv(d->Cout);
  p.M = d->N * Hin * Win; p.N = d->Cin; p.K = d->KH * d->KW * d->Cout;
  p.C = dx; p.ldc = d->Cin;
  return nk_gemm_dispatch(p, NK_OP_KCG, NK_OP_MCT, 0, 0, (hipStream_t)stream);
}

extern "C" long nk_conv2d_dgrad_flipped_ok(const NkConvDesc* d) {
  if (check_conv(d) || d->KH != 3 || d->KW != 3 || d->stride != 1 || d->pad_t != 1 || d->pad_l != 1) return 0;
  const int Hin = d->upsample ? 2 * d->H : d->H, Win = d->upsample ? 2 * d->W : d->W;
  if (d->Ho != Hin || d->Wo != Win) return 0;
  NkConvDesc t = *d;
  t.H = Hin; t.W = Win; t.Cin = d->Cout; t.Cout = d->Cin; t.upsample = 0;
  NkGemmParams p = conv_fwd_params(&t, nullptr, nullptr, nullptr, nullptr, nullptr, nullptr);
  return nk_halo_tiles_per_image(p, nullptr) > 0;
}

extern "C" int nk_conv2d_dgrad_flipped(const NkConvDesc* d, const void* dy, const void* wt, void* dx, void* stream) {
  NK_CHECK_ARG(nk_conv2d_dgrad_flipped_ok(d) == 1);
  const int Hin = d->upsample ? 2 * d->H : d->H, Win = d->upsample ? 2 * d->W : d->W;
  NkConvDesc t = *d;
  t.H = Hin; t.W = Win; t.Cin = d->Cout; t.Cout = d->Cin; t.upsample = 0;
  NkGemmParams p = conv_fwd_params(&t, dy, wt, nullptr, nullptr, nullptr, dx);
  return nk_gemm_dispatch(p, NK_OP_KCG, NK_OP_KC, 0, 0, (hipStream_t)stream);
}

static int conv_wgrad(const NkConvDesc* d, const void* dy, const void* x, float* dw, float* dbias, int accumulate, void* stream) {
  if (int e = check_conv(d)) return e;
  NkGemmParams p = zero_params();
  p.A = (const bf16_t*)dy; p.lda = d->Cout;
  p.B = (const bf16_t*)x; p.gb = fwd_gather(d);
  p.M = d->Cout; p.N = d->KH * d->KW * d->Cin; p.K = d->N * d->Ho * d->Wo;
  p.C = dw; p.ldc = p.N;
  p.accumulate = accumulate;
  p.dbias = dbias;
  p.halo_nb = (d->KH == 3 && d->KW == 3) ? d->N : 0;
  return nk_gemm_dispatch(p, NK_OP_MC, NK_OP_MCG, 1, 1, (hipStream_t)stream);
}
extern "C" int nk_conv2d_wgrad(const NkConvDesc* d, const void* dy, const void* x, float* dw, int accumulate,
                               void* stream) {
  return conv_wgrad(d, dy, x, dw, nullptr, accumulate, stream);
}
extern "C" int nk_conv2d_wgrad_bias(const NkConvDesc* d, const void* dy, const void* x, float* dw, float* dbias, int accumulate,
                                    void* stream) {
  NK_CHECK_ARG(dbias != nullptr);
  return conv_wgrad(d, dy, x, dw, dbias, accumulate, stream);
}

static int check_up2(const NkConvDesc* d) {
  if (int e = check_conv(d)) return e;
  NK_CHECK_ARG(d->upsample == 1 && d->KH == 3 && d->KW == 3 && d->stride == 1 && d->pad_t == 1 && d->pad_l == 1);
  NK_CHECK_ARG(d->Ho == 2 * d->H && d->Wo == 2 * d->W);
  return NK_OK;
}
static NkConvDesc up2_phase_desc(const NkConvDesc* d, int phase) {
  NkConvDesc t = *d;
  t.KH = t.KW = 2; t.pad_t = 1 - (phase >> 1); t.pad_l = 1 - (phase & 1);
  t.Ho = d->H; t.Wo = d->W; t.upsample = 0;
  return t;
}
static size_t up2_align(size_t b) { return (b + 255) & ~(size_t)255; }
static size_t up2_phase_image_bytes(const NkConvDesc* d) { return up2_align((size_t)4 * d->N * d->H * d->W * d->Cout * sizeof(bf16_t)); }
static size_t up2_phase_wgrad_bytes(const NkConvDesc* d) { return up2_align((size_t)16 * d->Cout * d->Cin * sizeof(float)); }

extern "C" long nk_conv2d_up2_ws_bytes(const NkConvDesc* d, int direction) {
  if (check_up2(d) || direction < 0 || direction > 2) return -1;
  if (direction == 0) return (long)up2_phase_image_bytes(d);
  if (direction == 1) return 0;
  return (long)(up2_phase_image_bytes(d) + up2_phase_wgrad_bytes(d) + up2_align((size_t)4 * d->Cout * sizeof(float)));
}

extern "C" int nk_conv2d_up2_fwd(const NkConvDesc* d, const void* x, const void* wp, const float* bias, void* y, void* ws, void* stream) {
  if (int e = check_up2(d)) return e;
  NK_CHECK_ARG(x && wp && y && ws && nk_aligned16(ws));
  const size_t img = (size_t)d->N * d->H * d->W * d->Cout;
  for (int ph = 0; ph < 4; ++ph) {
    const NkConvDesc t = up2_phase_desc(d, ph);
    NkGemmParams p = conv_fwd_params(&t, x, (const bf16_t*)wp + (size_t)ph * d->Cout * 4 * d->Cin, bias, nullptr, nullptr, (bf16_t*)ws + ph * img);
    if (int e = nk_gemm_dispatch(p, NK_OP_KCG, NK_OP_KC, 0, 0, (hipStream_t)stream)) return e;
  }
  if (nk_launch_log_mode() == 3) return NK_OK;
  return nk_pixel_shuffle2x(ws, y, d->N, d->H, d->W, d->Cout, stream);
}

extern "C" int nk_conv2d_up2_dgrad(const NkConvDesc* d, const void* dy, const void* wd, void* dx, void* stream) {
  if (int e = check_up2(d)) return e;
  NK_CHECK_ARG(dy && wd && dx);
  NkConvDesc t = *d;
  t.H = 2 * d->H; t.W = 2 * d->W; t.Cin = d->Cout; t.Cout = d->Cin;
  t.KH = t.KW = 4; t.stride = 2; t.Ho = d->H; t.Wo = d->W; t.upsample = 0;
  if (int e = check_conv(&t)) return e;
  NkGemmParams p = conv_fwd_params(&t, dy, wd, nullptr, nullptr, nullptr, dx);
  return nk_gemm_dispatch(p, NK_OP_KCG, NK_OP_KC, 0, 0, (hipStream_t)stream);
}

static int conv_up2_wgrad(const NkConvDesc* d, const void* dy, const void* x, float* dw, float* dbias, int accumulate, void* ws, void* stream) {
  if (int e = check_up2(d)) return e;
  NK_CHECK_ARG(dy && x && dw && ws && nk_aligned16(ws) && accumulate >= 0 && accumulate <= 2);
  const int plan_only = nk_launch_log_mode() == 3;
  bf16_t* dyp = (bf16_t*)ws;
  float* dwp = (float*)((char*)ws + up2_phase_image_bytes(d));
  float* dbp = dbias ? (float*)((char*)dwp + up2_phase_wgrad_bytes(d)) : nullptr;
  if (!plan_only)
    if (int e = nk_pixel_unshuffle2x(dy, dyp, d->N, d->H, d->W, d->Cout, stream)) return e;
  const size_t img = (size_t)d->N * d->H * d->W * d->Cout;
  for (int ph = 0; ph < 4; ++ph) {
    const NkConvDesc t = up2_phase_desc(d, ph);
// ... 14 lines not shown
```

neurosis_amd/lib.py:

```python
from __future__ import annotations

import ctypes as C
import os
from pathlib import Path

import torch

CSRC = Path(__file__).resolve().parent / "csrc"
LIB_PATH = CSRC / "libneurosis_hip.so"

vp, i32, i64, f32 = C.c_void_p, C.c_int, C.c_long, C.c_float


class NkConvDesc(C.Structure):
    _fields_ = [(n, i32) for n in ("N", "H", "W", "Cin", "Cout", "KH", "KW", "stride", "pad_t", "pad_l", "Ho", "Wo", "upsample")]


class NkAttnDesc(C.Structure):
    _fields_ = (
        [(n, i32) for n in ("B", "H", "Lq", "Lk", "D")]
        + [(n, i64) for n in ("sq", "sk", "sv", "so", "bq", "bk", "bv", "bo", "sdq", "sdk", "sdv", "sdo", "bdq", "bdk", "bdv", "bdo")]
        + [("scale", f32), ("causal", i32)]
    )


NK_COLPART_MAX = 32


class NkColpartBatch(C.Structure):
    _fields_ = [("part", vp * NK_COLPART_MAX), ("dgamma", vp * NK_COLPART_MAX), ("dbeta", vp * NK_COLPART_MAX), ("nrows", i32 * NK_COLPART_MAX),
                ("C", i32 * NK_COLPART_MAX), ("accumulate", i32 * NK_COLPART_MAX), ("n", i32)]


cdp, adp = C.POINTER(NkConvDesc), C.POINTER(NkAttnDesc)

SIGNATURES: dict[str, list] = {
    "nk_linear_fwd": [vp, vp, vp, vp, vp, i32, i32, i32, i64, i64, i64, i64, f32, vp],
    "nk_linear_dgrad": [vp, vp, vp, vp, i32, i32, i32, i64, i64, i64, i64, vp],
    "nk_linear_dgrad_geglu": [vp, vp, vp, vp, i32, i32, i32, i64, i64, i64, i64, vp],
    "nk_linear_fwd_geglu": [vp, vp, vp, vp, vp, i32, i32, i32, i64, i64, i64, i64, vp],
    "nk_linear_fwd_geglu_s": [vp, vp, vp, vp, vp, i32, i32, i32, i64, i64, i64, i64, vp],
    "nk_linear_dgrad_geglu_s": [vp, vp, vp, vp, i32, i32, i32, i64, i64, i64, i64, vp],
    "nk_linear_wgrad": [vp, vp, vp, i32, i32, i32, i64, i64, i64, i32, vp],
    "nk_linear_fwd_batched": [C.POINTER(vp), C.POINTER(vp), C.POINTER(vp), i32, i32, i32, i32, i64, i64, i64, vp],
    "nk_linear_wgrad_batched": [C.POINTER(vp), C.POINTER(vp), C.POINTER(vp), C.POINTER(vp), i32, i32, i32, i32, i64, i64, i64, i32, vp],
    "nk_linear_wgrad_bias": [vp, vp, vp, vp, i32, i32, i32, i64, i64, i64, i32, vp],
    "nk_conv2d_wgrad_bias": [cdp, vp, vp, vp, vp, i32, vp],
    "nk_conv2d_fwd": [cdp, vp, vp, vp, vp, vp, vp, vp],
    "nk_conv2d_fwd_stats": [cdp, vp, vp, vp, vp, vp, vp, vp, i32, vp],
    "nk_conv_weight_flip": [vp, vp, i32, i32, i32, vp],
    "nk_conv3x3_few_channels_fwd": [vp, vp, vp, vp, i32, i32, i32, i32, i32, vp],
    "nk_conv2d_dgrad": [cdp, vp, vp, vp, vp],
    "nk_conv2d_dgrad_flipped": [cdp, vp, vp, vp, vp],
    "nk_conv2d_wgrad": [cdp, vp, vp, vp, i32, vp],
    "nk_up2_phase_weights": [vp, vp, vp, i32, i32, vp],
    "nk_conv2d_up2_fwd": [cdp, vp, vp, vp, vp, vp, vp],
    "nk_conv2d_up2_dgrad": [cdp, vp, vp, vp, vp],
    "nk_conv2d_up2_wgrad": [cdp, vp, vp, vp, i32, vp, vp],
    "nk_conv2d_up2_wgrad_bias": [cdp, vp, vp, vp, vp, i32, vp, vp],
    "nk_pixel_shuffle2x": [vp, vp, i32, i32, i32, i32, vp],
    "nk_pixel_unshuffle2x": [vp, vp, i32, i32, i32, i32, vp],
    "nk_up2_fold_wgrad": [vp, vp, vp, vp, i32, i32, i32, vp],
    "nk_attention_fwd": [adp, vp, vp, vp, vp, vp, vp],
    "nk_attention_bwd": [adp, vp, vp, vp, vp, vp, vp, vp, vp, vp, vp, vp],
    "nk_attention_bwd_causal": [adp, vp, vp, vp, vp, vp, vp, vp, vp, vp, vp],
    "nk_attention_relbias_fwd": [adp, vp, vp, vp, vp, vp, vp],
    "nk_attention_relbias_fwd_lse": [adp, vp, vp, vp, vp, vp, vp, vp],
    "nk_attention_relbias_bwd": [adp, vp, vp, vp, vp, vp, vp, vp, vp, vp, vp, vp, vp, i32, vp],
    "nk_relbias_bucket_sum": [vp, vp, vp, i32, i32, i32, i32, vp],
    "nk_softmax_rows": [vp, i64, i32, vp],
    "nk_softmax_rows_bwd": [vp, vp, i64, i32, f32, vp],
    "nk_groupnorm_fwd": [vp, vp, vp, vp, vp, vp, vp, i32, i32, i32, i32, f32, i32, vp],
    "nk_groupnorm_sums": [vp, vp, vp, i32, i32, i32, i32, vp],
    "nk_groupnorm_sums_from_parts": [vp, vp, vp, i32, i32, i32, vp],
    "nk_groupnorm_apply": [vp, vp, vp, vp, vp, vp, vp, i32, i32, i32, i32, f32, i32, vp],
    "nk_groupnorm_bwd": [vp, vp, vp, vp, vp, vp, vp, vp, vp, vp, vp, i32, i32, i32, i32, i32, i32, vp],
    "nk_groupnorm_mod_fwd": [vp, vp, vp, vp, vp, vp, vp, vp, i32, i32, i32, i32, f32, i32, vp],
    "nk_groupnorm_mod_apply": [vp, vp, vp, vp, vp, vp, vp, vp, i32, i32, i32, i32, f32, i32, vp],
    "nk_groupnorm_mod_bwd": [vp, vp, vp, vp, vp, vp, vp, vp, vp, vp, vp, vp, vp, i32, i32, i32, i32, i32, i32, vp],
    "nk_layernorm_fwd": [vp, vp, vp, vp, vp, vp, i32, i32, f32, vp],
    "nk_rmsnorm_fwd": [vp, vp, vp, i32, i32, f32, vp],
    "nk_rmsnorm_fwd_rstd": [vp, vp, vp, vp, i32, i32, f32, vp],
    "nk_rmsnorm_bwd": [vp, vp, vp, vp, vp, vp, vp, vp, i32, i32, i32, vp],
    "nk_layernorm_bwd": [vp, vp, vp, vp, vp, vp, vp, vp, vp, vp, i32, i32, i32, vp],
    "nk_layernorm_bwd_dx": [vp, vp, vp, vp, vp, vp, vp, i32, i32, vp],
    "nk_layernorm_bwd_rows": [vp, vp, vp, vp, vp, vp, vp, vp, i32, i32, vp],
    "nk_colpart_reduce_batch": [C.POINTER(NkColpartBatch), vp],
    "nk_layernorm_bwd_params": [vp, vp, vp, vp, vp, vp, vp, i32, i32, i32, vp],
    "nk_geglu_fwd": [vp, vp, i64, i32, vp],
    "nk_geglu_bwd": [vp, vp, vp, i64, i32, vp],
    "nk_geglu_fwd_s": [vp, vp, vp, i64, i32, vp],
    "nk_geglu_bwd_s": [vp, vp, vp, i64, i32, vp],
    "nk_silu_fwd": [vp, vp, i64, vp],
    "nk_gelu_fwd": [vp, vp, i64, i32, vp],
    "nk_gated_gelu_tanh_fwd": [vp, vp, i64, i32, vp],
    "nk_gelu_bwd": [vp, vp, vp, i64, i32, vp],
    "nk_act_bwd": [vp, vp, vp, i64, i32, vp],
    "nk_gated_gelu_tanh_bwd": [vp, vp, vp, i64, i32, vp],
    "nk_embedding_bwd": [vp, vp, i64, vp, vp, i32, i32, i32, i32, i32, i32, vp],
    "nk_gather_rows_bwd": [vp, i64, vp, vp, i32, i32, i32, vp],
    "nk_wgrad_few_rows": [vp, i64, vp, i64, vp, i64, i32, i32, i32, i32, vp],
    "nk_vq_search": [vp, i64, vp, vp, vp, i64, i32, i32, vp],
    "nk_vq_code_stats": [vp, vp, i64, vp, vp, i64, i32, i32, vp],
    "nk_vq_quantize": [vp, vp, vp, i64, vp, vp, vp, i64, i32, i32, i32, vp],
    "nk_gumbel_logits": [vp, i64, vp, vp, vp, i64, i64, i32, i32, vp],
    "nk_gumbel_noise": [vp, i64, i32, vp, i32, vp],
    "nk_gumbel_softmax_fwd": [vp, i64, vp, vp, i32, f32, vp, vp, vp, vp, i64, i32, vp],
    "nk_gumbel_softmax_bwd": [vp, i64, vp, vp, f32, f32, i64, i32, vp],
    "nk_resample_planes": [vp, vp, vp, vp, vp, vp, i32, vp, vp, vp, i32, i64, i32, i32, i32, i32, vp],
    "nk_vit_patchify": [vp, vp, vp, i32, i32, i32, i32, vp],
    "nk_vit_patchify_bwd": [vp, vp, vp, vp, i32, i32, i32, i32, i32, vp],
    "nk_vit_tokens": [vp, vp, vp, vp, i32, i32, i32, vp],
    "nk_vit_tokens_bwd": [vp, vp, i32, i32, i32, vp],
    "nk_vit_add_ln": [vp, vp, vp, vp, vp, i32, vp, vp, vp, i32, i32, f32, vp],
    "nk_vit_cls_head_fwd": [vp, i64, vp, vp, vp, vp, vp, vp, vp, i32, i32, i32, f32, vp],
    "nk_vit_cls_head_bwd": [vp, vp, i64, vp, vp, vp, vp, vp, i32, i32, i32, vp],
    "nk_dreamsim_head_fwd": [vp, vp, i32, i32, f32, vp],
    "nk_dreamsim_head_bwd": [vp, vp, vp, i32, i32, f32, vp],
    "nk_leaky_relu_fwd": [vp, vp, i64, f32, vp],
    "nk_leaky_relu_bwd": [vp, vp, vp, i64, f32, vp],
    "nk_maxpool2x2_fwd": [vp, vp, i32, i32, i32, i32, vp],
    "nk_maxpool2x2_bwd": [vp, vp, vp, i32, i32, i32, i32, vp],
    "nk_maxpool_fwd": [vp, vp, i32, i32, i32, i32, i32, i32, vp],
    "nk_maxpool_bwd": [vp, vp, vp, i32, i32, i32, i32, i32, i32, vp],
    "nk_lpips_layer_fwd": [vp, vp, vp, vp, vp, i32, i32, i32, f32, i32, vp],
    "nk_lpips_layer_bwd": [vp, vp, vp, vp, vp, i32, i32, i32, f32, vp],
    "nk_batchnorm_fwd": [vp, vp, vp, vp, vp, vp, vp, vp, vp, i64, i32, f32, f32, f32, vp],
    "nk_batchnorm_bwd": [vp, vp, vp, vp, vp, vp, vp, vp, vp, vp, i64, i32, f32, i32, vp],
    "nk_batchnorm_eval": [vp, vp, vp, vp, vp, vp, vp, i64, i32, f32, f32, vp],
    "nk_silu_bwd": [vp, vp, vp, i64, vp],
    "nk_add": [vp, vp, vp, i64, vp],
    "nk_dropout": [vp, vp, vp, i64, i32, i64, i64, i64, vp, i32, i32, f32, vp],
    "nk_dropout_draw": [vp, vp, vp],
    "nk_cat_channels": [vp, vp, vp, i64, i32, i32, vp],
    "nk_split_channels": [vp, vp, vp, i64, i32, i32, vp],
    "nk_upsample2x_bwd": [vp, vp, i32, i32, i32, i32, vp],
    "nk_upsample2x_fwd": [vp, vp, i32, i32, i32, i32, vp],
    "nk_avgpool2x_fwd": [vp, vp, i32, i32, i32, i32, vp],
    "nk_avgpool2x_bwd": [vp, vp, i32, i32, i32, i32, vp],
    "nk_nchw_to_nhwc": [vp, i32, vp, i32, i32, i32, i32, f32, vp],
    "nk_nhwc_to_nchw": [vp, vp, i32, i32, i32, i32, i32, vp],
    "nk_cast_f32_to_bf16": [vp, vp, i64, vp],
    "nk_cast_bf16_to_f32": [vp, vp, i64, vp],
    "nk_colsum": [vp, vp, vp, i64, i32, i64, i32, vp],
    "nk_colsum_batched": [vp, vp, vp, i64, i32, i64, i32, i32, vp],
    "nk_timestep_embedding": [vp, vp, i32, i32, f32, vp],
    "nk_edm_prepare": [vp, vp, vp, vp, vp, vp, i32, i32, i32, i32, vp],
    "nk_edm_prepare_cat": [vp, vp, vp, vp, vp, vp, vp, i32, i32, i32, i32, i32, vp],
    "nk_edm_loss": [vp, vp, vp, vp, vp, vp, vp, vp, i32, i32, i32, i32, f32, vp],
    "nk_sample_prepare": [vp, vp, vp, i32, i32, i32, i32, i32, vp],
    "nk_sample_prepare_cat": [vp, vp, vp, vp, vp, i32, i32, i32, i32, i32, i32, vp],
    "nk_sample_denoise": [vp, vp, vp, vp, f32, vp, i32, i32, i32, i32, i32, vp],
    "nk_sample_euler_step": [vp, vp, vp, vp, vp, vp, f32, vp, vp, i32, i32, i32, i32, i32, vp],
    "nk_adamw_flat": [vp, vp, vp, vp, vp, i64, f32, f32, f32, f32, f32, i32, f32, vp],
    "nk_ema_flat": [vp, vp, i64, f32, vp],
    "nk_debug_raise_health": [vp],
    "nk_debug_stamp": [vp, vp],
    "nk_debug_launch_log": [i32],
    "nk_health_clear": [],
    "nk_health_export": [vp, vp],
    "nk_health_import": [vp, vp],
    "nk_adafactor_init": [vp, vp],
    "nk_adafactor_chunk": [vp, vp],
    "nk_adafactor_chunk_momentum": [vp, vp, f32, vp],
    "nk_came_chunk": [vp, vp],
    "nk_adamw8bit_step": [vp, vp],
}

SIZE_QUERIES: dict[str, list] = {
    "nk_groupnorm_ws_floats": [i32, i32, i32, i32],
    "nk_groupnorm_sums_ws_floats": [i32, i32, i32],
    "nk_conv2d_stats_tiles": [cdp, i32],
    "nk_conv2d_dgrad_flipped_ok": [cdp],
    "nk_conv2d_up2_ws_bytes": [cdp, i32],
    "nk_linear_fwd_geglu_ok": [i32, i32, i32],
    "nk_layernorm_ws_floats": [i32, i32],
    "nk_layernorm_part_rows": [i32],
    "nk_colsum_ws_floats": [i64, i32],
    "nk_batchnorm_ws_floats": [i64, i32],
    "nk_lpips_layer_ws_floats": [i32, i32],
    "nk_attention_bwd_ws_floats": [adp],
    "nk_attention_relbias_bwd_ws_floats": [adp],
    "nk_rmsnorm_bwd_ws_floats": [i32, i32],
    "nk_vq_search_ws_floats": [i64, i32],
    "nk_vq_quantize_ws_floats": [i64],
    "nk_gumbel_softmax_ws_floats": [i64],
    "nk_resample_ws_floats": [i64, i32, i32, i32, i32],
    "nk_adafactor_tensor_bytes": [],
    "nk_came_tensor_bytes": [],
    "nk_adamw8bit_tensor_bytes": [],
    "nk_gemm_sk_status": [],
    "nk_health_status": [],
    "nk_debug_launch_names": [C.c_char_p, i64],
}

_lib = None


class NkError(RuntimeError):
    pass


def load() -> C.CDLL:
    global _lib
    if _lib is not None:
        return _lib
    path = Path(os.environ.get("NEUROSIS_HIP_LIB", LIB_PATH))
    if not path.exists():
        raise NkError(
            f"{path} not found: the HIP extension is not built. Run `python -c 'import __graft_entry__ as g; g.build()'` "
            "(or `make -C neurosis_amd/csrc`). There is no CPU fallback for the product path."
        )
    lib = C.CDLL(str(path))
    lib.nk_last_error.restype = C.c_char_p
    lib.nk_last_error.argtypes = []
    lib.nk_abi_version.restype = i32
    lib.nk_abi_version.argtypes = []
    for name, argtypes in SIGNATURES.items():
        fn = getattr(lib, name)
        fn.argtypes = argtypes
        fn.restype = i32
    for name, argtypes in SIZE_QUERIES.items():
        fn = getattr(lib, name)
        fn.argtypes = argtypes
        fn.restype = i64
    _lib = lib
    return lib


def launch_log(mode: int) -> None:
    call("nk_debug_launch_log", int(mode))


def launched() -> list[str]:
    buf = C.create_string_buffer(8192)
    n = query("nk_debug_launch_names", buf, len(buf))
    if n < 0:
        raise NkError("nk_debug_launch_names failed")
    return buf.value.decode().split("\n")[:-1]


def query(name: str, *args) -> int:
    return int(getattr(load(), name)(*args))


def call(name: str, *args) -> None:
    lib = load()
    rc = getattr(lib, name)(*args)
    if rc != 0:
        raise NkError(f"{name} failed (rc={rc}): {lib.nk_last_error().decode()}")
```

neurosis_amd/modules/diffusion/openaimodel.py:

```python
from __future__ import annotations

import os

from typing import Callable, List, Optional, Union

import torch
from torch import Tensor, nn

from ... import ops
from ...nn import Conv2d, FlatParamStore, apply_module, as_tokens, linear_module_fwd
from ...ops import BF16, Img
from ..attention import SpatialTransformer, zero_module


def conv_nd(dims: int, *args, **kwargs) -> nn.Module:
    if dims != 2:
        raise ValueError(f"unsupported dimensions: {dims} (the MI355X path implements 2-D convolutions)")
    return Conv2d(*args, **kwargs)


class TimestepBlock(nn.Module):

    def forward(self, x: Tensor, emb: Tensor):
        raise NotImplementedError("TimestepBlock is an interface: subclasses implement forward(x, emb)")
# ... 131 lines not shown
            raise NotImplementedError("ResBlock: exchange_temb_dims / skip_t_emb are options of the video UNet, which is not on the MI355X path")
        self.channels = channels
        self.emb_channels = emb_channels
        self.dropout = self.dropout_p = ops.check_dropout_rate(dropout, "ResBlock")
        self.out_channels = out_channels if out_channels is not None else channels
        self.use_conv = use_conv
        self.use_checkpoint = use_checkpoint
        self.use_scale_shift_norm = use_scale_shift_norm
        self.exchange_temb_dims = exchange_temb_dims
        padding = kernel_size // 2
        self.in_layers = nn.Sequential(nn.GroupNorm(32, channels), nn.SiLU(), conv_nd(dims, channels, self.out_channels, kernel_size, padding=padding))
        self.updown = up or down
        self._up, self._down = bool(up), bool(down) and not up
        if up:
            self.h_upd = Upsample(channels, False, dims)
            self.x_upd = Upsample(channels, False, dims)
        elif down:
            self.h_upd = Downsample(channels, False, dims)
            self.x_upd = Downsample(channels, False, dims)
        else:
            self.h_upd = self.x_upd = nn.Identity()
        self.skip_t_emb = skip_t_emb
        self.emb_out_channels = 2 * self.out_channels if use_scale_shift_norm else self.out_channels
        self.emb_layers = nn.Sequential(nn.SiLU(), nn.Linear(emb_channels, self.emb_out_channels))
        self.out_layers = nn.Sequential(
            nn.GroupNorm(32, self.out_channels), nn.SiLU(), nn.Dropout(p=dropout),
            zero_module(conv_nd(dims, self.out_channels, self.out_channels, kernel_size, padding=padding)),
        )
        if self.out_channels == channels:
            self.skip_connection = nn.Identity()
        elif use_conv:
            self.skip_connection = conv_nd(dims, channels, self.out_channels, kernel_size, padding=padding)
        else:
            self.skip_connection = conv_nd(dims, channels, self.out_channels, 1)

    def _skip_fwd(self, x: Img):
        skip = self.skip_connection
        b_res = None
        if self._down:
            x, b_res = ops.avgpool2x_fwd(x)
        if isinstance(skip, nn.Identity):
            s, b_skip = x.t, None
        elif skip.kernel_size == 1:
            s, b_skip = ops.linear_fwd(x.t, skip.weight, skip.bias)
        else:
            si, b_skip3 = skip.fwd(x, upsample=self._up)
            s, b_skip = si.t, (lambda g: b_skip3(g)[0].t)
        b_up = None
        if self._up and (b_skip is None or skip.kernel_size == 1):
            sup, b_up = ops.upsample2x_fwd(Img(s, x.N, x.H, x.W))
            s = sup.t
        if b_skip is None and b_res is None and b_up is None:
            return s, None

        def bwd(dy: Tensor) -> Tensor:
            if b_up is not None:
                dy = b_up(dy)
            if b_skip is not None:
                dy = b_skip(dy)
            return dy if b_res is None else b_res(dy)

        return s, bwd

    def _fwd(self, x: Img, emb: Tensor):
        gn1, gn2 = self.in_layers[0], self.out_layers[0]
        ssn = self.use_scale_shift_norm
        h1, b_gn1 = ops.groupnorm_fwd(x, gn1.weight, gn1.bias, 32, gn1.eps, silu=True)
        b_pool = None
        if self._down:
            h1, b_pool = ops.avgpool2x_fwd(h1)
        es, b_es = ops.silu_fwd(emb)
        eo, b_eo = linear_module_fwd(self.emb_layers[1], es)
        h2, b_c1 = self.in_layers[2].fwd(h1, rowvec=None if ssn else eo, upsample=self._up, stats_groups=32)
        if ssn:
            h3, b_gn2 = ops.groupnorm_mod_fwd(h2, gn2.weight, gn2.bias, eo, 32, gn2.eps, silu=True)
        else:
            h3, b_gn2 = ops.groupnorm_fwd(h2, gn2.weight, gn2.bias, 32, gn2.eps, silu=True)
        b_drop = None
        if self.training and self.dropout_p > 0.0:
            _, b_drop = ops.dropout_fwd(h3.t, self.dropout_p, ops.dropout_site(self), inplace=True)
        s, b_skip = self._skip_fwd(x)
        out, b_c2 = self.out_layers[3].fwd(h3, residual=s, stats_groups=32)

        def bwd(dy: Tensor):
            dh3, _ = b_c2(dy)
            dh2 = b_gn2(dh3.t if b_drop is None else b_drop(dh3.t, inplace=True))
            if ssn:
                dh2, deo = dh2
                dh1, _ = b_c1(dh2)
            else:
                dh1, deo = b_c1(dh2)
            dh1 = dh1.t if b_pool is None else b_pool(dh1.t)
            dxs = dy if b_skip is None else b_skip(dy)
            dx = b_gn1(dh1, dxs)
            demb = b_es(b_eo(deo))
            return dx, demb

        return out, bwd

    def fwd(self, x: Img, emb: Tensor):
        if not (self.use_checkpoint and ops.recording()):
            return self._fwd(x, emb)
        out, _ = self._fwd(x, emb)
        tok = ops.dropout_token(required=False)

        def bwd(dy: Tensor):
            with ops.dropout_token_scope(tok):
                _, b = self._fwd(x, emb)
            return b(dy)

        return out, bwd

    def forward(self, x: Tensor, emb: Tensor) -> Tensor:
        ops.dropout_open(self)

        def run(x, emb):
            img = Img.from_nchw(x)
            out, bwd = self.fwd(img, as_tokens(emb))

            def bwd2(g):
                dx, demb = bwd(Img.from_nchw(g).t)
                return Img(dx, img.N, img.H, img.W).to_nchw(), demb.view(emb.shape)

            return out.to_nchw(), bwd2

        return apply_module(run, [x, emb], self)


class Timestep(nn.Module):

    def __init__(self, dim: int):
        super().__init__()
        self.dim = dim

    def forward(self, t: Tensor) -> Tensor:
        return ops.timestep_embedding(t, self.dim)


class UNetModel(nn.Module):

    def __init__(
        self,
        in_channels: int,
        model_channels: int,
        out_channels: int,
        num_res_blocks: int,
        attention_resolutions,
        dropout: float = 0.0,
        channel_mult=(1, 2, 4, 8),
        conv_resample: bool = True,
        dims: int = 2,
        num_classes=None,
        use_checkpoint: bool = False,
        num_heads: int = -1,
        num_head_channels: int = -1,
        num_heads_upsample: int = -1,
        use_scale_shift_norm: bool = False,
        resblock_updown: bool = False,
        transformer_depth=1,
        context_dim: Optional[int] = None,
        disable_self_attentions: Optional[List[bool]] = None,
        num_attention_blocks: Optional[List[int]] = None,
        disable_middle_self_attn: bool = False,
        disable_middle_transformer: bool = False,
        use_linear_in_transformer: bool = False,
        spatial_transformer_attn_type: str = "softmax",
        adm_in_channels: Optional[int] = None,
    ):
        super().__init__()
        if num_heads_upsample == -1:
            num_heads_upsample = num_heads
        if num_heads == -1:
            assert num_head_channels != -1, "UNetModel: num_heads = -1 needs num_head_channels"
        if num_head_channels == -1:
            assert num_heads != -1, "UNetModel: num_head_channels = -1 needs num_heads"
        self.in_channels = in_channels
        self.model_channels = model_channels
# ... 269 lines not shown
```

neurosis_amd/ops.py:

```python
from __future__ import annotations

import ctypes as C
import math
import os
import threading
import weakref
from dataclasses import dataclass
from typing import Callable, Optional

import torch
from torch import Tensor

from . import lib
from .lib import NkAttnDesc, NkConvDesc, call, query

BF16 = torch.bfloat16


class EngineState:

    _live = weakref.WeakSet()

    def __init__(self, wgrad_stream=None):
        self.grad_accumulate = False
# ... 123 lines not shown
                        continue
                    n = len(chunk)
                    arr = C.c_void_p * n
                    call("nk_linear_wgrad_batched", arr(*[c[0].data_ptr() for c in chunk]), arr(*[c[1].data_ptr() for c in chunk]),
                         arr(*[c[2].data_ptr() for c in chunk]), arr(*[None if c[3] is None else c[3].data_ptr() for c in chunk]), n, M, N, K,
                         lddy, ldx, lddw, mode, _stream())

        on_wgrad_stream(run, *[t for it in items for t in it[:2]], owner=self.owner)


def colpart_reduce(entries) -> None:
    for i in range(0, len(entries), lib.NK_COLPART_MAX):
        chunk = entries[i:i + lib.NK_COLPART_MAX]
        b = lib.NkColpartBatch()
        for z, (part, dgamma, dbeta, nrows, Cc, acc) in enumerate(chunk):
            b.part[z], b.dgamma[z], b.dbeta[z] = part.data_ptr(), dgamma.data_ptr(), dbeta.data_ptr()
            b.nrows[z], b.C[z], b.accumulate[z] = nrows, Cc, int(acc)
        b.n = len(chunk)
        call("nk_colpart_reduce_batch", C.byref(b), _stream())


_wgrad_queue: Optional[WgradQueue] = None


class batched_wgrads:

    def __init__(self, owner=None):
        self.owner = owner

    def __enter__(self):
        global _wgrad_queue
        self.prev = _wgrad_queue
        _wgrad_queue = WgradQueue(self.owner) if state_of(self.owner).batch_wgrads else None
        return _wgrad_queue

    def __exit__(self, *exc):
        global _wgrad_queue
        q, _wgrad_queue = _wgrad_queue, self.prev
        if exc[0] is None and q is not None:
            q.flush()
        return False


def join_wgrad_stream(owner=None) -> None:
    if owner is not None:
        st = state_of(owner)
        side = st.wgrad_stream
        if side is not None and st.deferred is None:
            torch.cuda.current_stream().wait_stream(side)
        return
    seen = set()
    for st in list(EngineState._live):
        side = st.wgrad_stream
        if side is not None and st.deferred is None and id(side) not in seen:
            seen.add(id(side))
            torch.cuda.current_stream().wait_stream(side)


def _ws(n_floats: int, device) -> Tensor:
    return torch.empty(n_floats, dtype=torch.float32, device=device)


def _p(t: Optional[Tensor]):
    return None if t is None else t.data_ptr()


def _stream():
    return torch.cuda.current_stream().cuda_stream


def _check2d(t: Tensor, name: str):
    if t.dim() != 2 or t.stride(1) != 1 or t.dtype != BF16 or not t.is_cuda:
        raise ValueError(f"{name}: expected a 2-D bf16 CUDA tensor with unit inner stride, got {tuple(t.shape)} {t.dtype} {t.stride()} {t.device}")


@dataclass
class Img:

    t: Tensor
    N: int
    H: int
    W: int
    sums: Optional[Tensor] = None

    @property
    def C(self) -> int:
        return self.t.shape[1]

    @staticmethod
    def from_nchw(x: Tensor) -> "Img":
        N, Cc, H, W = x.shape
        if x.dtype == BF16 and x.permute(0, 2, 3, 1).is_contiguous():
            return Img(x.permute(0, 2, 3, 1).reshape(N * H * W, Cc), N, H, W)
        return Img(nchw_to_tokens(x, Cc), N, H, W)

    def to_nchw(self) -> Tensor:
        return self.t.view(self.N, self.H, self.W, self.C).permute(0, 3, 1, 2)


def _param_stamp(p: Tensor):
    st = getattr(p, "_nk_store", None)
    if st is not None:
        return ("epoch", id(st), st.epoch)
    return ("version", p._version, p.data_ptr())


def shadow(p: Tensor) -> Tensor:
    if getattr(p, "_nk_store", None) is not None:
        return p._nk_shadow
    s = getattr(p, "_nk_shadow", None)
    stamp = _param_stamp(p)
    if s is not None and getattr(p, "_nk_shadow_stamp", None) == stamp:
        return s
    flat = _phys_flat(p)
    n = flat.numel()
    if s is not None and n % 8 == 0 and s.numel() == n and s.device == p.device:
        call("nk_cast_f32_to_bf16", flat.data_ptr(), s.data_ptr(), n, _stream())
        p._nk_shadow_stamp = stamp
        return s
    s = torch.empty(flat.numel(), dtype=BF16, device=p.device)
    if n % 8 == 0:
        call("nk_cast_f32_to_bf16", flat.data_ptr(), s.data_ptr(), n, _stream())
    else:
        pad = torch.zeros((n + 7) // 8 * 8, dtype=torch.float32, device=p.device)
        pad[:n] = flat
        s8 = torch.empty(pad.numel(), dtype=BF16, device=p.device)
        call("nk_cast_f32_to_bf16", pad.data_ptr(), s8.data_ptr(), pad.numel(), _stream())
        s = s8[:n]
    p._nk_shadow = s
    p._nk_shadow_stamp = stamp
    return s


def _phys_flat(p: Tensor) -> Tensor:
    d = p.detach()
    if d.dim() == 4:
        d = d.permute(0, 2, 3, 1)
    if not d.is_contiguous():
        raise ValueError("parameter storage must be dense (conv weights in channels_last memory format)")
    return d.reshape(-1)


def grad_flat(p: Tensor) -> Tensor:
    if p.grad is None:
        g = torch.zeros_like(p, memory_format=torch.preserve_format)
        p.grad = g
    g = p.grad
    if g.dim() == 4:
        g = g.permute(0, 2, 3, 1)
    if not g.is_contiguous():
        raise ValueError("parameter .grad must share the parameter's physical layout")
    return g.reshape(-1)


def w2d(p: Tensor) -> Tensor:
    return shadow(p).view(p.shape[0], -1)


def g2d(p: Tensor) -> Tensor:
    return grad_flat(p).view(p.shape[0], -1)


def conv_weight_param(out_ch: int, in_ch: int, kh: int, kw: int) -> torch.nn.Parameter:
    base = torch.empty(out_ch, kh, kw, in_ch)
    return torch.nn.Parameter(base.permute(0, 3, 1, 2))

# ... 113 lines not shown
    return y, _linear_bwd(x if x_saved is None else x_saved, weight, bias, need_dx)


def geglu_save_enabled() -> bool:
    return os.environ.get("NK_GEGLU_SAVE", "1") != "0"


def linear_geglu_fwd(x: Tensor, weight: Tensor, bias: Optional[Tensor], x_saved=None, save_derivative: bool = False):
    _check2d(x, "x")
    M, K = x.shape
    I2 = weight.shape[0]
    I = I2 // 2
    wq = w2d(weight)
    if I2 % 2 == 0 and x.is_contiguous() and query("nk_linear_fwd_geglu_ok", M, I, K):
        u = torch.empty(M, I2, dtype=BF16, device=x.device)
        h = torch.empty(M, I, dtype=BF16, device=x.device)
        call("nk_linear_fwd_geglu_s" if save_derivative else "nk_linear_fwd_geglu", x.data_ptr(), wq.data_ptr(), _p(bias), u.data_ptr(), h.data_ptr(), M, I, K,
             x.stride(0), wq.stride(0), u.stride(0), h.stride(0), _stream())
    else:
        u = gemm_nt(x, wq, bias, None)
        if save_derivative:
            h = torch.empty(M, I, dtype=BF16, device=x.device)
            call("nk_geglu_fwd_s", u.data_ptr(), h.data_ptr(), u.data_ptr(), M, I, _stream())
        else:
            h = geglu_fwd(u)[0]
    return u, h, _linear_bwd(x if x_saved is None else x_saved, weight, bias, True)


def _linear_bwd(x_in, weight: Tensor, bias: Optional[Tensor], need_dx: bool):
    def bwd(dy: Tensor, dx_add: Optional[Tensor] = None, geglu_u: Optional[Tensor] = None, geglu_s: Optional[Tensor] = None):
        entry = "nk_linear_dgrad_geglu"
        if geglu_s is not None:
            if geglu_u is not None:
                raise ValueError("linear bwd: geglu_u and geglu_s are exclusive")
            geglu_u, entry = geglu_s, "nk_linear_dgrad_geglu_s"
        x = x_in() if callable(x_in) else x_in
        queued = _wgrad_queue is not None and _wgrad_queue.takes(weight) and dy.is_contiguous() and x.is_contiguous()
        db = grad_flat(bias) if bias is not None else None
        if queued:
            _wgrad_queue.add(dy, x, g2d(weight), db)
        else:
            on_wgrad_stream(lambda: gemm_tn_f32(dy, x, g2d(weight), wgrad_mode(weight), dbias=db), dy, x, owner=weight)
        if not need_dx:
            return None
        if geglu_u is not None:
            if dx_add is not None:
                raise ValueError("linear bwd: geglu_u and dx_add are exclusive")
            M, N = dy.shape
            K = weight.shape[1]
            _check2d(geglu_u, "geglu_u")
            if geglu_u.shape != (M, 2 * K):
                raise ValueError(f"linear bwd: geglu_u must be [{M}, {2 * K}], got {tuple(geglu_u.shape)}")
            du = torch.empty(M, 2 * K, dtype=BF16, device=dy.device)
            wq = w2d(weight)
            call(entry, dy.data_ptr(), wq.data_ptr(), geglu_u.data_ptr(), du.data_ptr(), M, N, K, dy.stride(0), wq.stride(0),
                 geglu_u.stride(0), du.stride(0), _stream())
            return du
        return gemm_nn(dy, w2d(weight), dx_add)

    return bwd


def _conv_desc(N, H, W, Cin, Cout, KH, KW, stride, pad_t, pad_l, Ho, Wo, upsample) -> NkConvDesc:
    return NkConvDesc(N, H, W, Cin, Cout, KH, KW, stride, pad_t, pad_l, Ho, Wo, int(upsample))


def groupnorm_sums(x: Img, groups: int) -> Tensor:
    if x.sums is not None and x.sums.shape == (x.N, 2 * groups):
        return x.sums
    sums = torch.empty(x.N, 2 * groups, dtype=torch.float32, device=x.t.device)
    ws = _ws(query("nk_groupnorm_ws_floats", x.N, x.H * x.W, x.C, groups), x.t.device)
    call("nk_groupnorm_sums", x.t.data_ptr(), sums.data_ptr(), ws.data_ptr(), x.N, x.H * x.W, x.C, groups, _stream())
    return sums


UP2_PHASES_MIN_WORK = 1 << 28


def up2_phases_take(pixels: int, Cin: int, Cout: int) -> bool:
    mode = os.environ.get("NK_UP2_PHASES", "1")
    if mode == "0":
        return False
    return mode == "2" or pixels * Cin * Cout >= UP2_PHASES_MIN_WORK


def conv2d_fwd(x: Img, weight: Tensor, bias: Optional[Tensor], stride: int = 1, padding=1, upsample: bool = False,
               rowvec: Optional[Tensor] = None, residual: Optional[Tensor] = None, need_dx: bool = True,
               asym_pad: bool = False, stats_groups: Optional[int] = None, cin_real: Optional[int] = None):
    Cout, Cin, KH, KW = weight.shape
    if x.C != Cin:
        raise ValueError(f"conv2d: input has {x.C} channels, weight expects {Cin}")
    Hin, Win = (2 * x.H, 2 * x.W) if upsample else (x.H, x.W)
    if asym_pad:
        pad_t = pad_l = 0
        Ho = (Hin + 1 - KH) // stride + 1
        Wo = (Win + 1 - KW) // stride + 1
    else:
        pad_t = pad_l = int(padding)
        Ho = (Hin + 2 * pad_t - KH) // stride + 1
        Wo = (Win + 2 * pad_l - KW) // stride + 1
    d = _conv_desc(x.N, x.H, x.W, Cin, Cout, KH, KW, stride, pad_t, pad_l, Ho, Wo, upsample)
    y = torch.empty(x.N * Ho * Wo, Cout, dtype=BF16, device=x.t.device)
    _check2d(x.t, "x")
    if not x.t.is_contiguous():
        raise ValueError("conv2d: x must be dense channels-last")
    tiles = query("nk_conv2d_stats_tiles", C.byref(d), stats_groups) if stats_groups else 0
    sums_out = None
    up2 = (upsample and KH == 3 and KW == 3 and stride == 1 and pad_t == 1 and not asym_pad and rowvec is None and residual is None and not tiles
           and up2_phases_take(x.N * x.H * x.W, Cin, Cout))
    if tiles:
        dev = x.t.device
        part = torch.empty(x.N, tiles, 2 * stats_groups, dtype=torch.float32, device=dev)
        call("nk_conv2d_fwd_stats", C.byref(d), x.t.data_ptr(), w2d(weight).data_ptr(), _p(bias), _p(rowvec), _p(residual), y.data_ptr(),
             part.data_ptr(), stats_groups, _stream())
        sums_out = torch.empty(x.N, 2 * stats_groups, dtype=torch.float32, device=dev)
        ws = _ws(query("nk_groupnorm_sums_ws_floats", x.N, tiles, stats_groups), dev)
        call("nk_groupnorm_sums_from_parts", part.data_ptr(), sums_out.data_ptr(), ws.data_ptr(), x.N, tiles, stats_groups, _stream())
    elif (cin_real in (3, 4) and Cin == 8 and KH == 3 and KW == 3 and stride == 1 and pad_t == 1 and not asym_pad and not upsample and rowvec is None
          and residual is None and Cout % 8 == 0):
        call("nk_conv3x3_few_channels_fwd", x.t.data_ptr(), w2d(weight).data_ptr(), _p(bias), y.data_ptr(), x.N, x.H, x.W, Cout, cin_real, _stream())
    elif up2:
        dev = x.t.device
        wp = torch.empty(16 * Cout * Cin, dtype=BF16, device=dev)
        wd = torch.empty(16 * Cout * Cin, dtype=BF16, device=dev) if need_dx else None
        call("nk_up2_phase_weights", w2d(weight).data_ptr(), wp.data_ptr(), _p(wd), Cout, Cin, _stream())
        ws = torch.empty(query("nk_conv2d_up2_ws_bytes", C.byref(d), 0), dtype=torch.uint8, device=dev)
        call("nk_conv2d_up2_fwd", C.byref(d), x.t.data_ptr(), wp.data_ptr(), _p(bias), y.data_ptr(), ws.data_ptr(), _stream())
        del wp, ws
    else:
        call("nk_conv2d_fwd", C.byref(d), x.t.data_ptr(), w2d(weight).data_ptr(), _p(bias), _p(rowvec), _p(residual), y.data_ptr(), _stream())
    out = Img(y, x.N, Ho, Wo, sums_out)

    def up2_wgrad(dy: Tensor):
        ws = torch.empty(query("nk_conv2d_up2_ws_bytes", C.byref(d), 2), dtype=torch.uint8, device=dy.device)
        if bias is not None:
            call("nk_conv2d_up2_wgrad_bias", C.byref(d), dy.data_ptr(), x.t.data_ptr(), g2d(weight).data_ptr(), grad_flat(bias).data_ptr(), wgrad_mode(weight),
                 ws.data_ptr(), _stream())
        else:
            call("nk_conv2d_up2_wgrad", C.byref(d), dy.data_ptr(), x.t.data_ptr(), g2d(weight).data_ptr(), wgrad_mode(weight), ws.data_ptr(), _stream())

    def bwd(dy: Tensor):
        _check2d(dy, "dy")
        if not dy.is_contiguous():
            raise ValueError("conv2d bwd: dy must be dense")
        acc = state_of(weight).grad_accumulate

        if weight.requires_grad and up2:
            on_wgrad_stream(lambda: up2_wgrad(dy), dy, x.t, owner=weight)
        elif weight.requires_grad:
            if bias is not None:
                on_wgrad_stream(lambda: call("nk_conv2d_wgrad_bias", C.byref(d), dy.data_ptr(), x.t.data_ptr(), g2d(weight).data_ptr(), grad_flat(bias).data_ptr(),
                                             wgrad_mode(weight), _stream()), dy, x.t, owner=weight)
            else:
                on_wgrad_stream(lambda: call("nk_conv2d_wgrad", C.byref(d), dy.data_ptr(), x.t.data_ptr(), g2d(weight).data_ptr(), wgrad_mode(weight), _stream()),
                                dy, x.t, owner=weight)
        drow = None
        if rowvec is not None:
            drow32 = torch.empty(x.N, Cout, dtype=torch.float32, device=dy.device)
            ws = _ws(x.N * query("nk_colsum_ws_floats", Ho * Wo, Cout), dy.device)
            call("nk_colsum_batched", dy.data_ptr(), drow32.data_ptr(), ws.data_ptr(), Ho * Wo, Cout, dy.stride(0), x.N, 0, _stream())
            drow = cast_bf16(drow32)
        dx = None
        if need_dx and up2:
            dxt = torch.empty(x.N * x.H * x.W, Cin, dtype=BF16, device=dy.device)
            call("nk_conv2d_up2_dgrad", C.byref(d), dy.data_ptr(), wd.data_ptr(), dxt.data_ptr(), _stream())
            dx = Img(dxt, x.N, x.H, x.W)
        elif need_dx:
            dxt = torch.empty(x.N * Hin * Win, Cin, dtype=BF16, device=dy.device)
            if query("nk_conv2d_dgrad_flipped_ok", C.byref(d)):
                wt = torch.empty(Cin * 9 * Cout, dtype=BF16, device=dy.device)
                call("nk_conv_weight_flip", w2d(weight).data_ptr(), wt.data_ptr(), Cout, Cin, 9, _stream())
                call("nk_conv2d_dgrad_flipped", C.byref(d), dy.data_ptr(), wt.data_ptr(), dxt.data_ptr(), _stream())
            else:
                call("nk_conv2d_dgrad", C.byref(d), dy.data_ptr(), w2d(weight).data_ptr(), dxt.data_ptr(), _stream())
            if upsample:
                dsm = torch.empty(x.N * x.H * x.W, Cin, dtype=BF16, device=dy.device)
                call("nk_upsample2x_bwd", dxt.data_ptr(), dsm.data_ptr(), x.N, x.H, x.W, Cin, _stream())
                dxt = dsm
            dx = Img(dxt, x.N, x.H, x.W)
        return dx, drow

    return out, bwd


def groupnorm_fwd(x: Img, weight: Tensor, bias: Tensor, groups: int, eps: float, silu: bool, mod: Optional[Tensor] = None):
    what = "groupnorm" if mod is None else "groupnorm_mod"
    if not x.t.is_contiguous():
        raise ValueError(f"{what}: x must be dense channels-last")
    N, HW, Cc = x.N, x.H * x.W, x.C
    if mod is not None:
        _check2d(mod, "mod")
        if tuple(mod.shape) != (N, 2 * Cc) or not mod.is_contiguous():
            raise ValueError(f"groupnorm_mod: mod must be a dense [{N}, {2 * Cc}] (scale | shift) matrix, got {tuple(mod.shape)}")
    entry, mp = "nk_" + what, () if mod is None else (mod.data_ptr(),)
    y = torch.empty_like(x.t)
    mean = torch.empty(N, groups, dtype=torch.float32, device=x.t.device)
    rstd = torch.empty_like(mean)
    nws = query("nk_groupnorm_ws_floats", N, HW, Cc, groups)
    if x.sums is not None and x.sums.shape == (N, 2 * groups):
        call(entry + "_apply", x.t.data_ptr(), x.sums.data_ptr(), weight.data_ptr(), bias.data_ptr(), *mp, y.data_ptr(), mean.data_ptr(),
             rstd.data_ptr(), N, HW, Cc, groups, float(eps), int(silu), _stream())
    else:
        ws = _ws(nws, x.t.device)
        call(entry + "_fwd", x.t.data_ptr(), weight.data_ptr(), bias.data_ptr(), *mp, y.data_ptr(), mean.data_ptr(), rstd.data_ptr(),
             ws.data_ptr(), N, HW, Cc, groups, float(eps), int(silu), _stream())

    def bwd(dy: Tensor, dx_add: Optional[Tensor] = None):
        dx = torch.empty_like(x.t)
        dmod = () if mod is None else (torch.empty_like(mod),)
        ws2 = _ws(nws, dy.device)
        call(entry + "_bwd", dy.data_ptr(), x.t.data_ptr(), weight.data_ptr(), bias.data_ptr(), *mp, mean.data_ptr(), rstd.data_ptr(),
             _p(dx_add), dx.data_ptr(), grad_flat(weight).data_ptr(), grad_flat(bias).data_ptr(), *(t.data_ptr() for t in dmod), ws2.data_ptr(),
             N, HW, Cc, groups, int(silu), int(state_of(weight).grad_accumulate), _stream())
        return (dx, *dmod) if dmod else dx

    return Img(y, x.N, x.H, x.W), bwd


def groupnorm_mod_fwd(x: Img, weight: Tensor, bias: Tensor, mod: Tensor, groups: int, eps: float, silu: bool):
    if mod is None:
        raise ValueError("groupnorm_mod: mod is required")
    return groupnorm_fwd(x, weight, bias, groups, eps, silu, mod=mod)


def layernorm_fwd(x: Tensor, weight: Tensor, bias: Tensor, eps: float = 1e-5):
    _check2d(x, "x")
    if not x.is_contiguous():
        raise ValueError("layernorm: x must be dense")
    M, Cc = x.shape
    y = torch.empty_like(x)
    mean = torch.empty(M, dtype=torch.float32, device=x.device)
    rstd = torch.empty_like(mean)
    call("nk_layernorm_fwd", x.data_ptr(), weight.data_ptr(), bias.data_ptr(), y.data_ptr(), mean.data_ptr(), rstd.data_ptr(), M, Cc, float(eps), _stream())

    def bwd(dy: Tensor, dx_add: Optional[Tensor] = None):
        dx = torch.empty_like(x)
        acc = state_of(weight).grad_accumulate
        if os.environ.get("NK_LN_FUSED", "1") != "0":
            rows = query("nk_layernorm_part_rows", M)
            part = torch.empty(rows * 2 * Cc, dtype=torch.float32, device=dy.device)
            call("nk_layernorm_bwd_rows", dy.data_ptr(), x.data_ptr(), weight.data_ptr(), mean.data_ptr(), rstd.data_ptr(), _p(dx_add),
                 dx.data_ptr(), part.data_ptr(), M, Cc, _stream())
            entry = (part, grad_flat(weight), grad_flat(bias), rows, Cc, bool(acc))
            if _wgrad_queue is not None:
                _wgrad_queue.add_colpart(*entry)
            else:
                on_wgrad_stream(lambda: colpart_reduce([entry]), part, owner=weight)
            return dx
        ws = _ws(query("nk_layernorm_ws_floats", M, Cc), dy.device)
        call("nk_layernorm_bwd_dx", dy.data_ptr(), x.data_ptr(), weight.data_ptr(), mean.data_ptr(), rstd.data_ptr(), _p(dx_add),
             dx.data_ptr(), M, Cc, _stream())

        def params():
            call("nk_layernorm_bwd_params", dy.data_ptr(), x.data_ptr(), mean.data_ptr(), rstd.data_ptr(),
                 grad_flat(weight).data_ptr(), grad_flat(bias).data_ptr(), ws.data_ptr(), M, Cc, int(acc), _stream())

        st_ = state_of(weight)
        if st_.norm_params_on_side_stream if st_.norm_params_on_side_stream is not None else st_.deferred is not None:
            on_wgrad_stream(params, dy, x, mean, rstd, ws, owner=weight)
        else:
            params()
        return dx

    return y, bwd


def rmsnorm(x: Tensor, weight: Tensor, eps: float = 1e-6) -> Tensor:
    _check2d(x, "x")
    if not x.is_contiguous():
        raise ValueError("rmsnorm: x must be dense")
    M, Cc = x.shape
    if weight.dtype != torch.float32 or weight.numel() != Cc or not weight.is_contiguous():
        raise ValueError(f"rmsnorm: weight must be a dense fp32 vector of {Cc} elements, got {weight.dtype} {tuple(weight.shape)}")
    y = torch.empty_like(x)
    call("nk_rmsnorm_fwd", x.data_ptr(), weight.data_ptr(), y.data_ptr(), M, Cc, float(eps), _stream())
    return y


def rmsnorm_fwd(x: Tensor, weight: Tensor, eps: float = 1e-6):
    _check2d(x, "x")
    if not x.is_contiguous():
        raise ValueError("rmsnorm: x must be dense")
    M, Cc = x.shape
    if weight.dtype != torch.float32 or weight.numel() != Cc or not weight.is_contiguous():
        raise ValueError(f"rmsnorm: weight must be a dense fp32 vector of {Cc} elements, got {weight.dtype} {tuple(weight.shape)}")
    y = torch.empty_like(x)
    rstd = torch.empty(M, dtype=torch.float32, device=x.device)
    call("nk_rmsnorm_fwd_rstd", x.data_ptr(), weight.data_ptr(), y.data_ptr(), rstd.data_ptr(), M, Cc, float(eps), _stream())

    def bwd(dy: Tensor, dx_add: Optional[Tensor] = None) -> Tensor:
        if dy.shape != x.shape or dy.dtype != BF16 or not dy.is_contiguous():
            raise ValueError("rmsnorm bwd: dy must be a dense bf16 tensor of x's shape")
        if dx_add is not None and (dx_add.shape != x.shape or dx_add.dtype != BF16 or not dx_add.is_contiguous()):
            raise ValueError("rmsnorm bwd: dx_add must be a dense bf16 tensor of x's shape")
        dx = torch.empty_like(x)
        ws = _ws(query("nk_rmsnorm_bwd_ws_floats", M, Cc), x.device)
        call("nk_rmsnorm_bwd", dy.data_ptr(), x.data_ptr(), weight.data_ptr(), rstd.data_ptr(), _p(dx_add), dx.data_ptr(), grad_flat(weight).data_ptr(),
             ws.data_ptr(), M, Cc, int(state_of(weight).grad_accumulate), _stream())
# ... 986 lines not shown
```

Measured before the change: 26.40.

## Fuse GroupNorm-backward reduction sums into the 3x3 conv dgrad halo epilogue

Adds a third epilogue mode to the halo-tile conv kernel. While it writes the conv input gradient, the kernel also reads the GroupNorm input and computes per-channel partial sums of dz and dz*xhat, applying the SiLU derivative when needed. The GroupNorm backward then folds these per-tile partials instead of re-reading dy and x in a separate reduction pass. The aim is to remove one full read pass over the activation gradient and input in ResBlock backward, in exchange for extra epilogue work, register pressure and global-state arming between calls.

Result: no change. 26.41 (median of 6 runs) (+0.0%).

```diff
diff --git a/include/neurosis_hip.h b/include/neurosis_hip.h
--- a/include/neurosis_hip.h
+++ b/include/neurosis_hip.h
@@ -63,6 +63,10 @@
 int nk_conv_weight_flip(const void* w, void* wt, int Cout, int Cin, int taps, void* stream);
 long nk_conv2d_dgrad_flipped_ok(const NkConvDesc* d);
 int nk_conv2d_dgrad_flipped(const NkConvDesc* d, const void* dy, const void* wt, void* dx, void* stream);
+long nk_conv2d_gn_bwd_tiles(const NkConvDesc* d);
+long nk_conv2d_gn_bwd_pays(const NkConvDesc* d);
+int nk_conv2d_attach_gn_bwd_sums(const void* x, long ldx, const float* mean, const float* rstd, const float* gamma, const float* beta, int G,
+                                 int silu, float* chan_part);
 int nk_conv2d_dgrad(const NkConvDesc* d, const void* dy, const void* w, void* dx, void* stream);
 int nk_conv2d_wgrad(const NkConvDesc* d, const void* dy, const void* x, float* dw, int accumulate, void* stream);
 int nk_conv2d_wgrad_bias(const NkConvDesc* d, const void* dy, const void* x, float* dw, float* dbias, int accumulate, void* stream);
@@ -112,6 +116,9 @@
 int nk_groupnorm_bwd(const void* dy, const void* x, const float* gamma, const float* beta, const float* mean,
                      const float* rstd, const void* dx_add, void* dx, float* dgamma, float* dbeta, float* ws,
                      int N, int HW, int C, int G, int silu, int accumulate, void* stream);
+int nk_groupnorm_bwd_from_parts(const void* dy, const void* x, const float* gamma, const float* beta, const float* mean,
+                                const float* rstd, const void* dx_add, void* dx, float* dgamma, float* dbeta, float* ws,
+                                int N, int HW, int C, int G, int silu, int accumulate, const float* chan_part, int part_rows, void* stream);
 int nk_groupnorm_mod_fwd(const void* x, const float* gamma, const float* beta, const void* mod, void* y, float* mean, float* rstd,
                          float* ws, int N, int HW, int C, int G, float eps, int silu, void* stream);
 int nk_groupnorm_mod_apply(const void* x, const float* sums, const float* gamma, const float* beta, const void* mod, void* y, float* mean,
diff --git a/neurosis_amd/csrc/conv_halo.h b/neurosis_amd/csrc/conv_halo.h
--- a/neurosis_amd/csrc/conv_halo.h
+++ b/neurosis_amd/csrc/conv_halo.h
@@ -315,6 +315,14 @@
     mrow[i] = (img * H + y) * W + x;
   }
   bf16_t* const C = (bf16_t*)p.C;
+  auto lane16_sum = [](float x) {
+    x += __builtin_bit_cast(float, __builtin_amdgcn_update_dpp(0, __builtin_bit_cast(int, x), 0xB1, 0xF, 0xF, true));
+    x += __builtin_bit_cast(float, __builtin_amdgcn_update_dpp(0, __builtin_bit_cast(int, x), 0x4E, 0xF, 0xF, true));
+    x += __builtin_bit_cast(float, __builtin_amdgcn_update_dpp(0, __builtin_bit_cast(int, x), 0x141, 0xF, 0xF, true));
+    x += __builtin_bit_cast(float, __builtin_amdgcn_update_dpp(0, __builtin_bit_cast(int, x), 0x140, 0xF, 0xF, true));
+    return x;
+  };
+  if constexpr (STATS != 2) {
   uint4_t res8[MI][NJ / 2 ? NJ / 2 : 1];
   uint2_t res4[MI];
   if (p.residual) {
@@ -429,13 +437,6 @@
   if constexpr (STATS) {
     __syncthreads();
     float* const cs = (float*)ring;
-    auto lane16_sum = [](float x) {
-      x += __builtin_bit_cast(float, __builtin_amdgcn_update_dpp(0, __builtin_bit_cast(int, x), 0xB1, 0xF, 0xF, true));
-      x += __builtin_bit_cast(float, __builtin_amdgcn_update_dpp(0, __builtin_bit_cast(int, x), 0x4E, 0xF, 0xF, true));
-      x += __builtin_bit_cast(float, __builtin_amdgcn_update_dpp(0, __builtin_bit_cast(int, x), 0x141, 0xF, 0xF, true));
-      x += __builtin_bit_cast(float, __builtin_amdgcn_update_dpp(0, __builtin_bit_cast(int, x), 0x140, 0xF, 0xF, true));
-      return x;
-    };
 #pragma unroll
     for (int h = 0; h < NJ / 2; ++h)
 #pragma unroll
@@ -471,6 +472,128 @@
       p.stats_part[((long)img * per_img + trem) * 2 * p.stats_groups + 2 * (n0 / cpg + gi) + k] = a;
     }
   }
+  } else {
+    const int Gn = p.gnb_groups, cpg = Cout / Gn;
+    const bool silu = p.gnb_silu != 0;
+    constexpr bool XBATCH = !PROD;
+    uint4_t x8[MI][XBATCH && NJ / 2 ? NJ / 2 : 1];
+    uint2_t x4[MI];
+    auto load_x8 = [&](int i, int h) {
+      const int n = nb + h * 32 + (g4 & 1) * 16 + (g4 >> 1) * 8;
+      x8[i][XBATCH ? h : 0] = (mok[i] && n < Cout) ? *(const uint4_t*)(p.gnb_x + (long)mrow[i] * p.gnb_ldx + n) : (uint4_t){0u, 0u, 0u, 0u};
+    };
+#pragma unroll
+    for (int i = 0; i < MI; ++i) {
+      if constexpr (XBATCH) {
+#pragma unroll
+        for (int h = 0; h < NJ / 2; ++h) load_x8(i, h);
+      }
+      if constexpr (NJ & 1) {
+        const int n = nb + (NJ - 1) * 16 + g4 * 4;
+        x4[i] = (mok[i] && n < Cout) ? *(const uint2_t*)(p.gnb_x + (long)mrow[i] * p.gnb_ldx + n) : (uint2_t){0u, 0u};
+      }
+    }
+    auto coef = [&](int n, int cnt, float* mu, float* rs, float* ga, float* be) {
+      if (n < Cout) {
+        int g = n / cpg, rem = n - g * cpg;
+#pragma unroll
+        for (int e = 0; e < cnt; ++e) {
+          if (rem == cpg) { rem = 0; ++g; }
+          mu[e] = p.gnb_mean[img * Gn + g]; rs[e] = p.gnb_rstd[img * Gn + g];
+          ga[e] = p.gnb_gamma[n + e]; be[e] = p.gnb_beta[n + e];
+          ++rem;
+        }
+      } else {
+#pragma unroll
+        for (int e = 0; e < cnt; ++e) { mu[e] = 0.f; rs[e] = 0.f; ga[e] = 0.f; be[e] = 0.f; }
+      }
+    };
+    auto term = [&](float dzv, float xv, float mu, float rs, float ga, float be, float& a, float& b) {
+      const float xh = (xv - mu) * rs;
+      float d = dzv;
+      if (silu) d *= dsilu_f(xh * ga + be);
+      a += d;
+      b += d * xh;
+    };
+    __syncthreads();
+    float* const cs = (float*)ring;
+#pragma unroll
+    for (int h = 0; h < NJ / 2; ++h) {
+      const int n = nb + h * 32 + (g4 & 1) * 16 + (g4 >> 1) * 8;
+      float mu[8], rs[8], ga[8], be[8], sa[8], sb[8];
+      if constexpr (!XBATCH) {
+#pragma unroll
+        for (int i = 0; i < MI; ++i) load_x8(i, h);
+      }
+      coef(n, 8, mu, rs, ga, be);
+#pragma unroll
+      for (int e = 0; e < 8; ++e) { sa[e] = 0.f; sb[e] = 0.f; }
+#pragma unroll
+      for (int i = 0; i < MI; ++i) {
+        float v[8];
+#pragma unroll
+        for (int r = 0; r < 4; ++r) {
+          const float a_own = acc[i][2 * h][r], b_own = acc[i][2 * h + 1][r];
+          auto sw = __builtin_amdgcn_permlane16_swap(__float_as_uint(a_own), __float_as_uint(b_own), false, false);
+          v[r] = __uint_as_float(sw[0]);
+          v[4 + r] = __uint_as_float(sw[1]);
+        }
+#pragma unroll
+        for (int e = 0; e < 8; ++e) v[e] += 0.f;
+        const uint4_t packed = pack8(v);
+        const bool ok = mok[i] && n < Cout;
+        if (ok) *(uint4_t*)(C + (long)mrow[i] * p.ldc + n) = packed;
+        float q[8], fx[8];
+        unpack8(packed, q);
+        unpack8(x8[i][XBATCH ? h : 0], fx);
+#pragma unroll
+        for (int e = 0; e < 8; ++e) term(ok ? q[e] : 0.f, fx[e], mu[e], rs[e], ga[e], be[e], sa[e], sb[e]);
+      }
+#pragma unroll
+      for (int e = 0; e < 8; ++e) {
+        const float ta = lane16_sum(sa[e]), tb = lane16_sum(sb[e]);
+        const int col = h * 32 + (g4 & 1) * 16 + (g4 >> 1) * 8 + e;
+        if ((lane & 15) == 0) { cs[(wave * HN + col) * 2] = ta; cs[(wave * HN + col) * 2 + 1] = tb; }
+      }
+    }
+    if constexpr (NJ & 1) {
+      const int n = nb + (NJ - 1) * 16 + g4 * 4;
+      float mu[4], rs[4], ga[4], be[4], sa[4], sb[4];
+      coef(n, 4, mu, rs, ga, be);
+#pragma unroll
+      for (int e = 0; e < 4; ++e) { sa[e] = 0.f; sb[e] = 0.f; }
+#pragma unroll
+      for (int i = 0; i < MI; ++i) {
+        const float v[4] = {acc[i][NJ - 1][0] + 0.f, acc[i][NJ - 1][1] + 0.f, acc[i][NJ - 1][2] + 0.f, acc[i][NJ - 1][3] + 0.f};
+        uint2_t o;
+        o.x = pack2bf(v[0], v[1]);
+        o.y = pack2bf(v[2], v[3]);
+        const bool ok = mok[i] && n < Cout;
+        if (ok) *(uint2_t*)(C + (long)mrow[i] * p.ldc + n) = o;
+        float q[4], fx[4];
+        unpack4(o, q);
+        unpack4(x4[i], fx);
+#pragma unroll
+        for (int e = 0; e < 4; ++e) term(ok ? q[e] : 0.f, fx[e], mu[e], rs[e], ga[e], be[e], sa[e], sb[e]);
+      }
+#pragma unroll
+      for (int e = 0; e < 4; ++e) {
+        const float ta = lane16_sum(sa[e]), tb = lane16_sum(sb[e]);
+        const int col = (NJ - 1) * 16 + g4 * 4 + e;
+        if ((lane & 15) == 0) { cs[(wave * HN + col) * 2] = ta; cs[(wave * HN + col) * 2 + 1] = tb; }
+      }
+    }
+    __syncthreads();
+    if (tid < BN_ && n0 + tid < Cout) {
+      const int gh = tid / HN, cl = tid - gh * HN;
+      float a = 0.f, b = 0.f;
+#pragma unroll
+      for (int w4 = 0; w4 < 4; ++w4) { a += cs[((gh * 4 + w4) * HN + cl) * 2]; b += cs[((gh * 4 + w4) * HN + cl) * 2 + 1]; }
+      float* const row = p.gnb_chan_part + ((long)img * per_img + trem) * 2 * Cout;
+      row[n0 + tid] = b;
+      row[Cout + n0 + tid] = a;
+    }
+  }
 #ifdef NK_HALO_STAMPS
   asm volatile("s_waitcnt vmcnt(0)" ::: "memory");
   CH_STAMP(3);
diff --git a/neurosis_amd/csrc/gemm.hip b/neurosis_amd/csrc/gemm.hip
--- a/neurosis_amd/csrc/gemm.hip
+++ b/neurosis_amd/csrc/gemm.hip
@@ -1412,12 +1412,21 @@
 }
 
 static NkGemmKernel halo_kernel(const NkGemmPlan& pl) {
+  if (pl.flag == 2) {
+    if (pl.bn == 160) return pl.halo_rows == 8 ? nk_conv3x3_halo_kernel<160, 4, 2> : nk_conv3x3_halo_kernel<160, 2, 2>;
+    return pl.halo_rows == 8 ? nk_conv3x3_halo_kernel<128, 4, 2> : nk_conv3x3_halo_kernel<128, 2, 2>;
+  }
   if (pl.bn == 160) {
     if (pl.halo_rows == 8) return pl.flag ? nk_conv3x3_halo_kernel<160, 4, 1> : nk_conv3x3_halo_kernel<160, 4, 0>;
     return pl.flag ? nk_conv3x3_halo_kernel<160, 2, 1> : nk_conv3x3_halo_kernel<160, 2, 0>;
   }
   if (pl.halo_rows == 8) return pl.flag ? nk_conv3x3_halo_kernel<128, 4, 1> : nk_conv3x3_halo_kernel<128, 4, 0>;
   return pl.flag ? nk_conv3x3_halo_kernel<128, 2, 1> : nk_conv3x3_halo_kernel<128, 2, 0>;
+}
+
+static const char* halo_gnb_name(const NkGemmPlan& pl) {
+  if (pl.bn == 160) return pl.halo_rows == 8 ? "nk_conv3x3_halo_kernel<160,8,stats=2>" : "nk_conv3x3_halo_kernel<160,4,stats=2>";
+  return pl.halo_rows == 8 ? "nk_conv3x3_halo_kernel<128,8,stats=2>" : "nk_conv3x3_halo_kernel<128,4,stats=2>";
 }
 
 #include <mutex>
@@ -1492,8 +1501,24 @@
   return hipGetLastError() != hipSuccess ? NK_ERR_LAUNCH : NK_OK;
 }
 
+static thread_local NkGnBwdSums gnb_armed = {};
+void nk_gnb_arm(const NkGnBwdSums& a) { gnb_armed = a; }
+bool nk_gnb_take(NkGemmParams& p) {
+  const NkGnBwdSums a = gnb_armed;
+  gnb_armed = {};
+  if (!a.chan_part) return false;
+  p.gnb_x = a.x; p.gnb_ldx = a.ldx; p.gnb_mean = a.mean; p.gnb_rstd = a.rstd; p.gnb_gamma = a.gamma; p.gnb_beta = a.beta;
+  p.gnb_groups = a.groups; p.gnb_silu = a.silu; p.gnb_chan_part = a.chan_part;
+  return true;
+}
+
 int nk_gemm_dispatch(NkGemmParams& p, int amode, int bmode, int out_f32, int allow_splitk,
                      hipStream_t stream) {
+  if (gnb_armed.chan_part) {
+    gnb_armed = {};
+    nk_set_error(__FILE__, __LINE__, "GroupNorm-backward sums were attached, but the next tile-engine dispatch is not nk_conv2d_dgrad_flipped");
+    return NK_ERR_ARG;
+  }
   NK_CHECK_ARG(p.M > 0 && p.N > 0 && p.K > 0);
   if (!p.nbatch) NK_CHECK_ARG(((uintptr_t)p.A & 15) == 0 && ((uintptr_t)p.B & 15) == 0 && ((uintptr_t)p.C & 15) == 0);
   for (int z = 0; z < p.nbatch; ++z) NK_CHECK_ARG(((uintptr_t)p.Ab[z] & 15) == 0 && ((uintptr_t)p.Bb[z] & 15) == 0 && ((uintptr_t)p.Cb[z] & 15) == 0);
@@ -1517,11 +1542,12 @@
   }
 
   const TileEnv env = tile_env();
-  const NkGemmPlan pl = nk_gemm_plan(p, amode, bmode, out_f32, allow_splitk, env);
+  NkGemmPlan pl = nk_gemm_plan(p, amode, bmode, out_f32, allow_splitk, env);
   if (pl.err) {
     nk_set_error(__FILE__, __LINE__, pl.err);
     return NK_ERR_ARG;
   }
+  if (pl.family == NK_FAM_HALO && pl.flag == 2) pl.name = halo_gnb_name(pl);
   if (pl.zero_c) NK_CHECK_ARG(p.ldc == p.N);
   const int logging = nk_launch_log_mode();
   char line[192];
diff --git a/neurosis_amd/csrc/gemm_plan.h b/neurosis_amd/csrc/gemm_plan.h
--- a/neurosis_amd/csrc/gemm_plan.h
+++ b/neurosis_amd/csrc/gemm_plan.h
@@ -318,7 +318,7 @@
   static const char* const names[2][2][2] = {
       {{"nk_conv3x3_halo_kernel<128,4,stats=0>", "nk_conv3x3_halo_kernel<128,4,stats=1>"}, {"nk_conv3x3_halo_kernel<128,8,stats=0>", "nk_conv3x3_halo_kernel<128,8,stats=1>"}},
       {{"nk_conv3x3_halo_kernel<160,4,stats=0>", "nk_conv3x3_halo_kernel<160,4,stats=1>"}, {"nk_conv3x3_halo_kernel<160,8,stats=0>", "nk_conv3x3_halo_kernel<160,8,stats=1>"}}};
-  return names[bn == 160][rows == 8][stats != 0];
+  return names[bn == 160][rows == 8][stats == 1];
 }
 
 static NkGemmPlan nk_gemm_plan(const NkGemmParams& p, int amode, int bmode, int out_f32, int allow_splitk, const TileEnv& env) {
@@ -342,7 +342,7 @@
   }
   if (use_halo(env, p, amode, bmode, out_f32)) {
     const NkGather& g = p.ga;
-    pl.bn = halo_bn(p.N); pl.halo_rows = halo_tile_rows(p); pl.flag = p.stats_part != nullptr;
+    pl.bn = halo_bn(p.N); pl.halo_rows = halo_tile_rows(p); pl.flag = p.gnb_chan_part ? 2 : p.stats_part != nullptr;
     pl.tiles_per_image = cdiv(g.W, CH_TW) * cdiv(g.H, pl.halo_rows);
     plan_kernel(pl, NK_FAM_HALO, halo_name(pl.bn, pl.halo_rows, pl.flag), (long)p.halo_nb * pl.tiles_per_image * (p.N / pl.bn), 1, 1,
                 halo_threads(pl.bn), halo_smem(pl.bn, pl.halo_rows));
@@ -363,6 +363,10 @@
   }
   if (p.stats_part) {
     pl.err = "statistics epilogue on a convolution the halo-tile kernel does not take (ask nk_conv2d_stats_tiles first)";
+    return pl;
+  }
+  if (p.gnb_chan_part) {
+    pl.err = "GroupNorm-backward sums attached to an input gradient the halo-tile kernel does not take (ask nk_conv2d_gn_bwd_tiles first)";
     return pl;
   }
 
diff --git a/neurosis_amd/csrc/nk_gemm.h b/neurosis_amd/csrc/nk_gemm.h
--- a/neurosis_amd/csrc/nk_gemm.h
+++ b/neurosis_amd/csrc/nk_gemm.h
@@ -56,6 +56,11 @@
   int halo_nb;
   float* stats_part;
   int stats_groups;
+  const bf16_t* gnb_x;
+  long gnb_ldx;
+  const float *gnb_mean, *gnb_rstd, *gnb_gamma, *gnb_beta;
+  int gnb_groups, gnb_silu;
+  float* gnb_chan_part;
 };
 #define NK_MAX_BATCH 8
 
@@ -64,3 +69,12 @@
 int nk_gemm_dispatch(NkGemmParams& p, int amode, int bmode, int out_f32, int allow_splitk, hipStream_t stream);
 int nk_halo_tiles_per_image(const NkGemmParams& p, int* bn);
 int nk_geglu_fwd_fusable(const NkGemmParams& p);
+struct NkGnBwdSums {
+  const bf16_t* x;
+  long ldx;
+  const float *mean, *rstd, *gamma, *beta;
+  int groups, silu;
+  float* chan_part;
+};
+void nk_gnb_arm(const NkGnBwdSums& a);
+bool nk_gnb_take(NkGemmParams& p);
diff --git a/neurosis_amd/csrc/norm.hip b/neurosis_amd/csrc/norm.hip
--- a/neurosis_amd/csrc/norm.hip
+++ b/neurosis_amd/csrc/norm.hip
@@ -407,6 +407,53 @@
                                 float* dgamma, float* dbeta, float* ws, int N, int HW, int C, int G, int silu, int accumulate, void* stream) {
   return gn_backward(false, dy, x, gamma, beta, nullptr, mean, rstd, dx_add, dx, dgamma, dbeta, nullptr, ws, N, HW, C, G, silu, accumulate, stream);
 }
+__global__ __launch_bounds__(1024) void gn_bwd_fold_parts_kernel(const float* __restrict__ chan_part, const float* __restrict__ gamma, float* __restrict__ gsum,
+                                                                 int tiles, int C, int G) {
+  __shared__ float lanes[2][64];
+  const int g = blockIdx.x, n = blockIdx.y, cpg = C / G, tx = threadIdx.x & 63;
+  nk_reduce_rows<16, 64, 2, 0, 4>(
+      tx < cpg, tiles,
+      [&](int t, float* s) {
+        const float* row = chan_part + ((long)n * tiles + t) * 2 * C;
+        for (int c = g * cpg + tx; c < (g + 1) * cpg; c += 64) {
+          const float gc = gamma[c];
+          s[0] += gc * row[C + c];
+          s[1] += gc * row[c];
+        }
+      },
+      [&](const float* s) { lanes[0][tx] = s[0]; lanes[1][tx] = s[1]; });
+  __syncthreads();
+  if (threadIdx.x < 2) {
+    const int m = cpg < 64 ? cpg : 64;
+    float s = 0.f;
+    for (int j = 0; j < m; ++j) s += lanes[threadIdx.x][j];
+    gsum[((long)n * G + g) * 2 + threadIdx.x] = s;
+  }
+}
+
+extern "C" int nk_groupnorm_bwd_from_parts(const void* dy, const void* x, const float* gamma, const float* beta, const float* mean, const float* rstd, const void* dx_add,
+                                           void* dx, float* dgamma, float* dbeta, float* ws, int N, int HW, int C, int G, int silu, int accumulate,
+                                           const float* chan_part, int part_rows, void* stream_) {
+  hipStream_t stream = (hipStream_t)stream_;
+  const NkGnPlan p = nk_gn_bwd_parts_plan(N, HW, C, G, part_rows);
+  NORM_PLAN_OR_RETURN(p);
+  NK_CHECK_ARG(dy && x && gamma && beta && mean && rstd && dx && dgamma && dbeta && ws && chan_part);
+  float* gsum = ws + p.gsum.off;
+  for (int i = 0; i < p.n; ++i) {
+    const NkNormLaunch& L = p.launch[i];
+    switch (L.kernel) {
+      case NK_GN_BWD_FOLD: NORM_LAUNCH(L, gn_bwd_fold_parts_kernel, chan_part, gamma, gsum, part_rows, C, G); break;
+      case NK_GN_BWD_APPLY:
+        NORM_LAUNCH(L, gn_bwd_apply_kernel<false>, (const bf16_t*)dy, (const bf16_t*)x, gamma, beta, (const bf16_t*)nullptr, mean, rstd, gsum, (const bf16_t*)dx_add,
+                    (bf16_t*)dx, HW, C, G, silu, p.rows_per);
+        break;
+      case NK_GN_COLPART: NORM_LAUNCH(L, colpart_reduce_kernel, chan_part, dgamma, dbeta, p.chan_rows, C, accumulate); break;
+    }
+    if (int e = nk_check_launch(L.name)) return e;
+  }
+  return NK_OK;
+}
+
 extern "C" int nk_groupnorm_mod_fwd(const void* x, const float* gamma, const float* beta, const void* mod, void* y, float* mean, float* rstd, float* ws, int N, int HW,
                                     int C, int G, float eps, int silu, void* stream) {
   return gn_forward(GN_FWD, true, x, nullptr, gamma, beta, mod, y, mean, rstd, ws, N, HW, C, G, eps, silu, stream);
diff --git a/neurosis_amd/csrc/norm_plan.h b/neurosis_amd/csrc/norm_plan.h
--- a/neurosis_amd/csrc/norm_plan.h
+++ b/neurosis_amd/csrc/norm_plan.h
@@ -23,7 +23,7 @@
 enum NormKernel {
   NK_GN_STATS, NK_GN_REDUCE, NK_GN_REDUCE_L1, NK_GN_APPLY, NK_GN_BWD_STATS, NK_GN_COLPART, NK_GN_COLPART_MOD, NK_GN_DMOD, NK_GN_BWD_APPLY,
   NK_LN_FWD, NK_LN_BWD_DX, NK_LN_BWD_PARAM, NK_LN_BWD_ROWS, NK_LN_COLPART, NK_RMS_FWD, NK_COLPART_BATCH, NK_CS_PARTIAL, NK_CS_REDUCE,
-  NK_RMS_BWD_ROWS, NK_RMS_COLPART
+  NK_RMS_BWD_ROWS, NK_RMS_COLPART, NK_GN_BWD_FOLD
 };
 struct NkNormRegion { const char* name; long off, len; };
 struct NkNormLaunch {
@@ -107,6 +107,23 @@
     }
     norm_launch(p, NK_GN_BWD_APPLY, mod ? "gn_bwd_apply_kernel<mod>" : "gn_bwd_apply_kernel", ns, n, 1, GN_THREADS, 2 * smem2, p.gsum);
   }
+  return p;
+}
+
+static inline NkGnPlan nk_gn_bwd_parts_plan(int N, int HW, int C, int G, int part_rows) {
+  NkGnPlan p = nk_gn_plan(N, HW, C, G, GN_APPLY, false);
+  if (p.err) return p;
+  p.n = 0;
+  if (!(part_rows > 0 && (long)N * part_rows < (1l << 24))) { p.err = "part_rows > 0 && N * part_rows < 2^24"; return p; }
+  p.chan_rows = N * part_rows;
+  p.part = {"part", 0, 0};
+  p.gsum = {"gsum", 0, (long)N * 2 * G};
+  p.chan = {"chan", 0, 0};
+  p.ws_floats = p.gsum.len + NORM_WS_PAD;
+  const int smem2 = 2 * C * (int)sizeof(float);
+  norm_launch(p, NK_GN_BWD_FOLD, "gn_bwd_fold_parts_kernel", (unsigned)G, (unsigned)N, 1, 1024, 0, p.gsum);
+  norm_launch(p, NK_GN_BWD_APPLY, "gn_bwd_apply_kernel", (unsigned)p.nsplit, (unsigned)N, 1, GN_THREADS, 2 * smem2, p.gsum);
+  norm_launch(p, NK_GN_COLPART, "colpart_reduce_kernel", (unsigned)((C + 63) / 64), 1, 1, 1024, 0);
   return p;
 }
 
diff --git a/neurosis_amd/csrc/ops_gemm.hip b/neurosis_amd/csrc/ops_gemm.hip
--- a/neurosis_amd/csrc/ops_gemm.hip
+++ b/neurosis_amd/csrc/ops_gemm.hip
@@ -1,5 +1,6 @@
 #include "../../include/neurosis_hip.h"
 #include "nk_gemm.h"
+#include "norm_plan.h"
 #include <string.h>
 
 static NkGemmParams zero_params() {
@@ -255,12 +256,47 @@
 }
 
 extern "C" int nk_conv2d_dgrad_flipped(const NkConvDesc* d, const void* dy, const void* wt, void* dx, void* stream) {
+  NkGemmParams sums = zero_params();
+  const bool attached = nk_gnb_take(sums);
+  if (attached && nk_conv2d_gn_bwd_tiles(d) <= 0) {
+    nk_set_error(__FILE__, __LINE__, "GroupNorm-backward sums attached to an input gradient the halo-tile kernel does not take (ask nk_conv2d_gn_bwd_tiles first)");
+    return NK_ERR_ARG;
+  }
   NK_CHECK_ARG(nk_conv2d_dgrad_flipped_ok(d) == 1);
   const int Hin = d->upsample ? 2 * d->H : d->H, Win = d->upsample ? 2 * d->W : d->W;
   NkConvDesc t = *d;
   t.H = Hin; t.W = Win; t.Cin = d->Cout; t.Cout = d->Cin; t.upsample = 0;
   NkGemmParams p = conv_fwd_params(&t, dy, wt, nullptr, nullptr, nullptr, dx);
+  if (attached) {
+    NK_CHECK_ARG(sums.gnb_groups <= 64 && d->Cin % sums.gnb_groups == 0);
+    p.gnb_x = sums.gnb_x; p.gnb_ldx = sums.gnb_ldx; p.gnb_mean = sums.gnb_mean; p.gnb_rstd = sums.gnb_rstd; p.gnb_gamma = sums.gnb_gamma;
+    p.gnb_beta = sums.gnb_beta; p.gnb_groups = sums.gnb_groups; p.gnb_silu = sums.gnb_silu; p.gnb_chan_part = sums.gnb_chan_part;
+  }
   return nk_gemm_dispatch(p, NK_OP_KCG, NK_OP_KC, 0, 0, (hipStream_t)stream);
+}
+
+extern "C" long nk_conv2d_gn_bwd_tiles(const NkConvDesc* d) {
+  if (!nk_conv2d_dgrad_flipped_ok(d) || d->upsample) return 0;
+  NkConvDesc t = *d;
+  t.Cin = d->Cout; t.Cout = d->Cin;
+  NkGemmParams p = conv_fwd_params(&t, nullptr, nullptr, nullptr, nullptr, nullptr, nullptr);
+  return nk_halo_tiles_per_image(p, nullptr);
+}
+
+extern "C" long nk_conv2d_gn_bwd_pays(const NkConvDesc* d) {
+  if (nk_conv2d_gn_bwd_tiles(d) <= 0) return 0;
+  const NkGnPlan gp = nk_gn_plan(d->N, d->H * d->W, 8, 1, GN_BWD, false);
+  return !gp.err && (long)d->N * gp.nsplit <= 256 ? 1 : 0;
+}
+
+extern "C" int nk_conv2d_attach_gn_bwd_sums(const void* x, long ldx, const float* mean, const float* rstd, const float* gamma, const float* beta, int G, int silu,
+                                            float* chan_part) {
+  NkGnBwdSums none = {};
+  nk_gnb_arm(none);
+  NK_CHECK_ARG(x && mean && rstd && gamma && beta && chan_part && G > 0 && nk_aligned16(x) && (ldx & 7) == 0);
+  const NkGnBwdSums a = {(const bf16_t*)x, ldx, mean, rstd, gamma, beta, G, silu ? 1 : 0, chan_part};
+  nk_gnb_arm(a);
+  return NK_OK;
 }
 
 static int conv_wgrad(const NkConvDesc* d, const void* dy, const void* x, float* dw, float* dbias, int accumulate, void* stream) {
diff --git a/neurosis_amd/lib.py b/neurosis_amd/lib.py
--- a/neurosis_amd/lib.py
+++ b/neurosis_amd/lib.py
@@ -75,6 +75,8 @@
     "nk_groupnorm_sums_from_parts": [vp, vp, vp, i32, i32, i32, vp],
     "nk_groupnorm_apply": [vp, vp, vp, vp, vp, vp, vp, i32, i32, i32, i32, f32, i32, vp],
     "nk_groupnorm_bwd": [vp, vp, vp, vp, vp, vp, vp, vp, vp, vp, vp, i32, i32, i32, i32, i32, i32, vp],
+    "nk_groupnorm_bwd_from_parts": [vp, vp, vp, vp, vp, vp, vp, vp, vp, vp, vp, i32, i32, i32, i32, i32, i32, vp, i32, vp],
+    "nk_conv2d_attach_gn_bwd_sums": [vp, i64, vp, vp, vp, vp, i32, i32, vp],
     "nk_groupnorm_mod_fwd": [vp, vp, vp, vp, vp, vp, vp, vp, i32, i32, i32, i32, f32, i32, vp],
     "nk_groupnorm_mod_apply": [vp, vp, vp, vp, vp, vp, vp, vp, i32, i32, i32, i32, f32, i32, vp],
     "nk_groupnorm_mod_bwd": [vp, vp, vp, vp, vp, vp, vp, vp, vp, vp, vp, vp, vp, i32, i32, i32, i32, i32, i32, vp],
@@ -172,6 +174,8 @@
     "nk_groupnorm_sums_ws_floats": [i32, i32, i32],
     "nk_conv2d_stats_tiles": [cdp, i32],
     "nk_conv2d_dgrad_flipped_ok": [cdp],
+    "nk_conv2d_gn_bwd_tiles": [cdp],
+    "nk_conv2d_gn_bwd_pays": [cdp],
     "nk_conv2d_up2_ws_bytes": [cdp, i32],
     "nk_linear_fwd_geglu_ok": [i32, i32, i32],
     "nk_layernorm_ws_floats": [i32, i32],
diff --git a/neurosis_amd/modules/diffusion/openaimodel.py b/neurosis_amd/modules/diffusion/openaimodel.py
--- a/neurosis_amd/modules/diffusion/openaimodel.py
+++ b/neurosis_amd/modules/diffusion/openaimodel.py
@@ -237,17 +237,24 @@
         s, b_skip = self._skip_fwd(x)
         out, b_c2 = self.out_layers[3].fwd(h3, residual=s, stats_groups=32)
 
+        gn2_ctx = getattr(b_gn2, "ctx", None) if b_drop is None and not ssn and getattr(b_c2, "takes_gn", False) else None
+        gn1_ctx = getattr(b_gn1, "ctx", None) if b_pool is None and not self._up and getattr(b_c1, "takes_gn", False) else None
+
         def bwd(dy: Tensor):
-            dh3, _ = b_c2(dy)
-            dh2 = b_gn2(dh3.t if b_drop is None else b_drop(dh3.t, inplace=True))
+            dh3, _ = b_c2(dy) if gn2_ctx is None else b_c2(dy, gn=gn2_ctx)
+            if dh3.gn_bwd_parts is not None:
+                dh2 = b_gn2(dh3.t, parts=dh3.gn_bwd_parts)
+            else:
+                dh2 = b_gn2(dh3.t if b_drop is None else b_drop(dh3.t, inplace=True))
             if ssn:
                 dh2, deo = dh2
                 dh1, _ = b_c1(dh2)
             else:
-                dh1, deo = b_c1(dh2)
+                dh1, deo = b_c1(dh2) if gn1_ctx is None else b_c1(dh2, gn=gn1_ctx)
+            parts1 = dh1.gn_bwd_parts
             dh1 = dh1.t if b_pool is None else b_pool(dh1.t)
             dxs = dy if b_skip is None else b_skip(dy)
-            dx = b_gn1(dh1, dxs)
+            dx = b_gn1(dh1, dxs) if parts1 is None else b_gn1(dh1, dxs, parts=parts1)
             demb = b_es(b_eo(deo))
             return dx, demb
 
diff --git a/neurosis_amd/ops.py b/neurosis_amd/ops.py
--- a/neurosis_amd/ops.py
+++ b/neurosis_amd/ops.py
@@ -229,6 +229,7 @@
     H: int
     W: int
     sums: Optional[Tensor] = None
+    gn_bwd_parts: Optional[Tensor] = None
 
     @property
     def C(self) -> int:
@@ -508,6 +509,13 @@
     if mode == "0":
         return False
     return mode == "2" or pixels * Cin * Cout >= UP2_PHASES_MIN_WORK
+
+
+def gn_bwd_epilogue_tiles(d: NkConvDesc) -> int:
+    mode = os.environ.get("NK_GN_BWD_EPI", "1")
+    if mode == "0" or (mode != "2" and not query("nk_conv2d_gn_bwd_pays", C.byref(d))):
+        return 0
+    return query("nk_conv2d_gn_bwd_tiles", C.byref(d))
 
 
 def conv2d_fwd(x: Img, weight: Tensor, bias: Optional[Tensor], stride: int = 1, padding=1, upsample: bool = False,
@@ -565,7 +573,7 @@
         else:
             call("nk_conv2d_up2_wgrad", C.byref(d), dy.data_ptr(), x.t.data_ptr(), g2d(weight).data_ptr(), wgrad_mode(weight), ws.data_ptr(), _stream())
 
-    def bwd(dy: Tensor):
+    def bwd(dy: Tensor, gn=None):
         _check2d(dy, "dy")
         if not dy.is_contiguous():
             raise ValueError("conv2d bwd: dy must be dense")
@@ -593,9 +601,17 @@
             dx = Img(dxt, x.N, x.H, x.W)
         elif need_dx:
             dxt = torch.empty(x.N * Hin * Win, Cin, dtype=BF16, device=dy.device)
+            parts = None
             if query("nk_conv2d_dgrad_flipped_ok", C.byref(d)):
                 wt = torch.empty(Cin * 9 * Cout, dtype=BF16, device=dy.device)
                 call("nk_conv_weight_flip", w2d(weight).data_ptr(), wt.data_ptr(), Cout, Cin, 9, _stream())
+                tiles = gn_bwd_epilogue_tiles(d) if gn is not None else 0
+                if tiles:
+                    if gn["x"].shape != dxt.shape or gn["mean"].shape != (x.N, gn["groups"]):
+                        raise ValueError("conv2d bwd: gn is not the GroupNorm that produced this convolution's input")
+                    parts = torch.empty(x.N * tiles, 2 * Cin, dtype=torch.float32, device=dy.device)
+                    call("nk_conv2d_attach_gn_bwd_sums", gn["x"].data_ptr(), gn["x"].stride(0), gn["mean"].data_ptr(), gn["rstd"].data_ptr(),
+                         gn["weight"].data_ptr(), gn["bias"].data_ptr(), gn["groups"], int(gn["silu"]), parts.data_ptr())
                 call("nk_conv2d_dgrad_flipped", C.byref(d), dy.data_ptr(), wt.data_ptr(), dxt.data_ptr(), _stream())
             else:
                 call("nk_conv2d_dgrad", C.byref(d), dy.data_ptr(), w2d(weight).data_ptr(), dxt.data_ptr(), _stream())
@@ -603,9 +619,10 @@
                 dsm = torch.empty(x.N * x.H * x.W, Cin, dtype=BF16, device=dy.device)
                 call("nk_upsample2x_bwd", dxt.data_ptr(), dsm.data_ptr(), x.N, x.H, x.W, Cin, _stream())
                 dxt = dsm
-            dx = Img(dxt, x.N, x.H, x.W)
+            dx = Img(dxt, x.N, x.H, x.W, gn_bwd_parts=parts)
         return dx, drow
 
+    bwd.takes_gn = True
     return out, bwd
 
 
@@ -631,15 +648,25 @@
         call(entry + "_fwd", x.t.data_ptr(), weight.data_ptr(), bias.data_ptr(), *mp, y.data_ptr(), mean.data_ptr(), rstd.data_ptr(),
              ws.data_ptr(), N, HW, Cc, groups, float(eps), int(silu), _stream())
 
-    def bwd(dy: Tensor, dx_add: Optional[Tensor] = None):
+    def bwd(dy: Tensor, dx_add: Optional[Tensor] = None, parts: Optional[Tensor] = None):
         dx = torch.empty_like(x.t)
         dmod = () if mod is None else (torch.empty_like(mod),)
         ws2 = _ws(nws, dy.device)
+        if parts is not None:
+            if mod is not None or parts.shape[1] != 2 * Cc or parts.shape[0] % N:
+                raise ValueError("groupnorm bwd: parts do not belong to this GroupNorm")
+            call("nk_groupnorm_bwd_from_parts", dy.data_ptr(), x.t.data_ptr(), weight.data_ptr(), bias.data_ptr(), mean.data_ptr(), rstd.data_ptr(),
+                 _p(dx_add), dx.data_ptr(), grad_flat(weight).data_ptr(), grad_flat(bias).data_ptr(), ws2.data_ptr(), N, HW, Cc, groups, int(silu),
+                 int(state_of(weight).grad_accumulate), parts.data_ptr(), parts.shape[0] // N, _stream())
+            return dx
         call(entry + "_bwd", dy.data_ptr(), x.t.data_ptr(), weight.data_ptr(), bias.data_ptr(), *mp, mean.data_ptr(), rstd.data_ptr(),
              _p(dx_add), dx.data_ptr(), grad_flat(weight).data_ptr(), grad_flat(bias).data_ptr(), *(t.data_ptr() for t in dmod), ws2.data_ptr(),
              N, HW, Cc, groups, int(silu), int(state_of(weight).grad_accumulate), _stream())
         return (dx, *dmod) if dmod else dx
 
+    bwd.ctx = None
+    if mod is None:
+        bwd.ctx = {"x": x.t, "mean": mean, "rstd": rstd, "weight": weight, "bias": bias, "groups": groups, "silu": silu}
     return Img(y, x.N, x.H, x.W), bwd
 
 
```
